# rfonod/geo-trax

Measured on AMD Instinct MI355X. Metric: 4K frames/sec through detect+stabilize+track, higher is better.
Workload: dtype f32 (split-f16x3 MFMA)

## Files before the change

geo-trax_amd/csrc/conv_igemm_split.hip:

```cpp
#include <hip/hip_runtime.h>
#include <hip/hip_fp16.h>

#include <cmath>

#include "conv_split_device.hpp"

namespace gtx {

namespace {

#define GTXS_MFMA(a, b, c) __builtin_amdgcn_mfma_f32_32x32x16_f16(a, b, c, 0, 0, 0)

#ifndef GTXS_DIAG_LOOP_BEGIN
#define GTXS_DIAG_ENTRY()
#define GTXS_DIAG_LOOP_BEGIN()
#define GTXS_DIAG_LOOP_END()
#define GTXS_DIAG_EXIT()
#define GTXS_DIAG_PHASE(K)
#endif

template <int KS, int STRIDE, int WN, int CPR, int WM>
struct SplitTile {
  static constexpr int TH = 8 * WM, TW = 16;
  static constexpr int BN = 32 * WN;
  static constexpr int PAD = KS / 2;
  static constexpr int PH = (TH - 1) * STRIDE + KS;
  static constexpr int PW = (TW - 1) * STRIDE + KS;
  static constexpr int NPIX = PH * PW;
  static constexpr int NCH = 2 * CPR;
  static constexpr int RB = NCH * 16;
  static constexpr int KC = 8 * CPR;
  static constexpr int PATCH_UNITS = NPIX * CPR;
  static constexpr int PATCH_SLOTS = (PATCH_UNITS + 255) / 256;
  static constexpr int W_CHUNKS = KS * KS * BN * NCH;
  static constexpr int W_SLOTS = (W_CHUNKS + 255) / 256;
  static constexpr int PATCH_BYTES = NPIX * RB;
  static constexpr int STAGE_BYTES = PATCH_BYTES + KS * KS * BN * RB;
  static constexpr int EPI_PITCH = epi_pitch(BN), EPI_BYTES = epi_bytes(BN);
  static constexpr int LDS_BYTES = STAGE_BYTES > EPI_BYTES ? STAGE_BYTES : EPI_BYTES;
  static constexpr int ROWS_PER_BANKROW = 256 / RB;
  static __host__ __device__ constexpr int swz(int row) { return (row / ROWS_PER_BANKROW) & (NCH - 1); }
};

__device__ __forceinline__ floatx4 acc_group(const floatx16 a, const int g4) { return floatx4{a[4 * g4], a[4 * g4 + 1], a[4 * g4 + 2], a[4 * g4 + 3]}; }
__device__ __forceinline__ void set_acc_group(floatx16& a, const int g4, const floatx4 v) {
#pragma unroll
  for (int k = 0; k < 4; ++k) a[4 * g4 + k] = v[k];
}

struct FrontTile {
  static constexpr int PH = 17, PW = 33, NPIX = PH * PW;
  static constexpr int IH = 2 * PH + 1, IW = 2 * PW + 1;
  static constexpr int IN_PIX = IH * IW;
  static constexpr int IN_SLOTS = (IN_PIX + 255) / 256;
  static constexpr int IN_BYTES = IN_PIX * 16;
  static constexpr int TILES = (NPIX + 15) / 16;
  static constexpr int LUT_BYTES = 256 * 4;
};

template <int KS, int STRIDE, int WN, int CPR, int WM, int FRONT>
constexpr int split_lds_bytes() {
  using Tile = SplitTile<KS, STRIDE, WN, CPR, WM>;
  if (!FRONT) return Tile::LDS_BYTES;
  const int wreg = Tile::STAGE_BYTES - Tile::PATCH_BYTES > FrontTile::IN_BYTES ? Tile::STAGE_BYTES - Tile::PATCH_BYTES : FrontTile::IN_BYTES;
  const int stage = Tile::PATCH_BYTES + wreg;
  return (stage > Tile::EPI_BYTES ? stage : Tile::EPI_BYTES) + FrontTile::LUT_BYTES;
}

template <int KS, int STRIDE, int WN, int CPR, int WM>
constexpr int split_min_waves() {
  if (WM == 2) return 2;
  if (KS == 3) return STRIDE == 1 ? 3 : 2;
  return WN == 1 ? 5 : 4;
}

template <int KS, int STRIDE, int WN, int CPR, int WM, int FRONT>
__device__ __forceinline__ void conv_split_body(const ConvGroup& g) {
  using Tile = SplitTile<KS, STRIDE, WN, CPR, WM>;
  static_assert(!FRONT || (KS == 3 && STRIDE == 2 && WM == 1 && CPR == 2), "front stage: 3x3 stride 2, 16-channel chunks");
  constexpr int TH = Tile::TH, TW = Tile::TW, BN = Tile::BN, PW = Tile::PW, RB = Tile::RB, KC = Tile::KC;

  extern __shared__ __attribute__((aligned(16))) char smem[];
  char* lds_patch = smem;
  char* lds_w = smem + Tile::PATCH_BYTES;

  GTXS_DIAG_ENTRY()
  const int tid = threadIdx.x;
  const int lane = tid & 63;
  const int wave = __builtin_amdgcn_readfirstlane(tid >> 6);

  ConvProblem P;
  int ct, n, oy0, ox0;
  if (!conv_block_decode<TH, TW>(g, P, ct, n, oy0, ox0)) return;
  const int iy0 = oy0 * STRIDE - Tile::PAD, ix0 = ox0 * STRIDE - Tile::PAD;

  const float* __restrict__ in = static_cast<const float*>(P.in);
  const float* __restrict__ in2 = static_cast<const float*>(P.in2);
  const int nchunks = P.Cin / KC;
  constexpr int c_begin = 0;
  const int c_end = nchunks;

  long goff[Tile::PATCH_SLOTS];
  long goff2[Tile::PATCH_SLOTS];
  int loff[Tile::PATCH_SLOTS];
  int lchk[Tile::PATCH_SLOTS];
  if constexpr (FRONT == 0) {
#pragma unroll
  for (int s = 0; s < Tile::PATCH_SLOTS; ++s) {
    const int qid = tid + 256 * s;
    const int p = qid / CPR, c = qid % CPR;
    const int py = p / PW, px = p - py * PW;
    const int iy = iy0 + py, ix = ix0 + px;
    const bool used = qid < Tile::PATCH_UNITS;
    const bool inb = used && iy >= 0 && iy < P.H && ix >= 0 && ix < P.W;
    goff[s] = inb ? ((long)(n * P.H + iy) * P.W + ix) * P.in_cstride + P.in_coff + c * 8 : -1;
    goff2[s] = (KS == 1 && inb) ? ((long)(n * (P.H >> 1) + (iy >> 1)) * (P.W >> 1) + (ix >> 1)) * P.in2_cstride + P.in2_coff + c * 8 : -1;
    loff[s] = used ? p * RB + ((c ^ Tile::swz(p)) << 4) : -1;
    lchk[s] = used ? p * RB + (((CPR + c) ^ Tile::swz(p)) << 4) : -1;
  }
  }
  const uint4* __restrict__ wsrc =
      reinterpret_cast<const uint4*>(P.wpack) + (size_t)ct * nchunks * Tile::W_CHUNKS + tid;

  const int prow = lane & 31, h = lane >> 5;
  const int tcol = prow & 15;
  const int trow0 = 2 * WM * wave + (prow >> 4);
  const int p0 = trow0 * STRIDE * PW + tcol * STRIDE;
  constexpr int PSUB = 2 * STRIDE * PW;

  uint4 pre_a[Tile::PATCH_SLOTS], pre_b[Tile::PATCH_SLOTS];
  uint4 pre_w[Tile::W_SLOTS];
#define GTXS_PREFETCH(CHUNK)                                                                 \
  {                                                                                          \
    const int c0__ = (CHUNK) * KC;                                                           \
    const bool up__ = KS == 1 && c0__ < P.c_split;    \
    if constexpr (FRONT == 0) {                           \
    _Pragma("unroll") for (int s = 0; s < Tile::PATCH_SLOTS; ++s) {                          \
      uint4 va__ = make_uint4(0, 0, 0, 0), vb__ = make_uint4(0, 0, 0, 0);                    \
      if (goff[s] >= 0) {                                                                    \
        const uint4* src__ = reinterpret_cast<const uint4*>(up__ ? in2 + goff2[s] + c0__ : in + goff[s] + c0__); \
        va__ = src__[0];                                                                     \
        vb__ = src__[1];                                                                     \
      }                                                                                      \
      pre_a[s] = va__;                                                                       \
      pre_b[s] = vb__;                                                                       \
    }                                                                                        \
    }                                                                                        \
    const uint4* w__ = wsrc + (size_t)(CHUNK) * Tile::W_CHUNKS;                              \
    _Pragma("unroll") for (int s = 0; s < Tile::W_SLOTS; ++s) {                              \
      uint4 v__ = make_uint4(0, 0, 0, 0);                                                    \
      if (Tile::W_CHUNKS % 256 == 0 || tid + 256 * s < Tile::W_CHUNKS) v__ = w__[256 * s];  \
      pre_w[s] = v__;                                                                        \
    }                                                                                        \
  }
#define GTXS_COMMIT()                                                                        \
  {                                                                                          \
    if constexpr (FRONT == 0) {                                                                  \
    _Pragma("unroll") for (int s = 0; s < Tile::PATCH_SLOTS; ++s) {                          \
      if (loff[s] >= 0) {                               \
        *reinterpret_cast<uint4*>(lds_patch + loff[s]) = pre_a[s];                           \
        *reinterpret_cast<uint4*>(lds_patch + lchk[s]) = pre_b[s];                           \
      }                                                                                      \
    }                                                                                        \
    }                                                                                        \
    _Pragma("unroll") for (int s = 0; s < Tile::W_SLOTS; ++s) {                              \
      if (Tile::W_CHUNKS % 256 == 0 || tid + 256 * s < Tile::W_CHUNKS)                       \
        *reinterpret_cast<uint4*>(lds_w + (tid + 256 * s) * 16) = pre_w[s];                  \
    }                                                                                        \
  }

  constexpr int FN = FRONT > 0 ? FRONT : 1;
  unsigned f_raw[FrontTile::IN_SLOTS];
  uint2 f_wh[FN][3], f_wl[FN][3];
  float4 f_bias[FN];
  uint2 f_keep[FN > 1 ? FrontTile::TILES / 4 : 1][2];
  char* const f_stage = lds_w;
  unsigned* const f_lut = reinterpret_cast<unsigned*>(smem + split_lds_bytes<KS, STRIDE, WN, CPR, WM, FRONT>() - FrontTile::LUT_BYTES);
  int f_toff[3];
  if constexpr (FRONT > 0) {
    const unsigned* __restrict__ img = static_cast<const unsigned*>(P.front_img) + (size_t)n * P.front_h * P.front_w_px;
    const int gy0 = 2 * iy0 - 1, gx0 = 2 * ix0 - 1;
#pragma unroll
    for (int s = 0; s < FrontTile::IN_SLOTS; ++s) {
      const int i = tid + 256 * s;
      const int r = i / FrontTile::IW, c = i - r * FrontTile::IW;
      const int gy = gy0 + r, gx = gx0 + c;
      f_raw[s] = (i < FrontTile::IN_PIX && gy >= 0 && gy < P.front_h && gx >= 0 && gx < P.front_w_px) ? img[gy * P.front_w_px + gx] : 0u;
    }
#pragma unroll
    for (int c = 0; c < FN; ++c) {
      const uint2* fw = static_cast<const uint2*>(P.front_w) + (size_t)c * (3 * 2 * 64) + lane;
#pragma unroll
      for (int s = 0; s < 3; ++s) {
        f_wh[c][s] = fw[(2 * s + 0) * 64];
        f_wl[c][s] = fw[(2 * s + 1) * 64];
      }
      f_bias[c] = *reinterpret_cast<const float4*>(P.front_bias + c * KC + 4 * (lane >> 4));
    }
#pragma unroll
    for (int s = 0; s < 3; ++s) {
      const int tap = min(4 * s + (lane >> 4), 8);
      f_toff[s] = ((tap / 3) * FrontTile::IW + tap % 3) * 16;
    }
    {
      const float f = (float)tid / 255.f;
      const _Float16 hi = (_Float16)f, lo = (_Float16)(f - (float)hi);
      f_lut[tid] = (unsigned)__builtin_bit_cast(unsigned short, hi) | ((unsigned)__builtin_bit_cast(unsigned short, lo) << 16);
    }
  }
#define GTXS_FRONT_EPI(ACC, BIAS, HV, LV)                                                    \
  {                                                                                          \
     \
    float2v v__[2] = {silu2(__builtin_elementwise_fma(float2v{(ACC)[0], (ACC)[1]}, float2v{P.front_scale, P.front_scale}, float2v{(BIAS).x, (BIAS).y})), \
                      silu2(__builtin_elementwise_fma(float2v{(ACC)[2], (ACC)[3]}, float2v{P.front_scale, P.front_scale}, float2v{(BIAS).z, (BIAS).w}))}; \
    if (!in__) v__[0] = v__[1] = float2v{0.f, 0.f};                                          \
    bool sat__ = false;                                                                      \
    split4(v__, HV, LV, sat__);                                                              \
  }
#define GTXS_FRONT_PUT(T, HV, LV)                                                            \
  {                                                                                          \
    const int qq__ = min((wave + 4 * (T)) * 16 + (lane & 15), FrontTile::NPIX - 1);          \
    const int cg__ = lane >> 4;                               \
    char* row__ = lds_patch + qq__ * RB + (cg__ & 1) * 8;                                    \
    *reinterpret_cast<uint2*>(row__ + (((cg__ >> 1) ^ Tile::swz(qq__)) << 4)) = (HV);        \
    *reinterpret_cast<uint2*>(row__ + (((CPR + (cg__ >> 1)) ^ Tile::swz(qq__)) << 4)) = (LV); \
  }
#define GTXS_FRONT_STAGE()                                                                   \
  {                                                                                          \
    unsigned e__[FrontTile::IN_SLOTS][3];            \
    _Pragma("unroll") for (int s = 0; s < FrontTile::IN_SLOTS; ++s) {                        \
      const unsigned px__ = f_raw[s];                                                        \
      e__[s][0] = f_lut[px__ & 255u]; e__[s][1] = f_lut[(px__ >> 8) & 255u]; e__[s][2] = f_lut[(px__ >> 16) & 255u]; \
    }                                                                                        \
    _Pragma("unroll") for (int s = 0; s < FrontTile::IN_SLOTS; ++s) {                        \
      const int i__ = tid + 256 * s;                                                         \
      if (FrontTile::IN_PIX % 256 == 0 || i__ < FrontTile::IN_PIX)                           \
        *reinterpret_cast<uint4*>(f_stage + i__ * 16) =                                      \
            make_uint4((e__[s][0] & 0xffffu) | (e__[s][1] << 16), e__[s][2] & 0xffffu, (e__[s][0] >> 16) | (e__[s][1] & 0xffff0000u), e__[s][2] >> 16); \
    }                                                                                        \
    __syncthreads();                                                                         \
  }
#define GTXS_FRONT_X(T)                               \
  {                                                                                          \
    const int qc__ = min((wave + 4 * (T)) * 16 + (lane & 15), FrontTile::NPIX - 1);    \
    const int py__ = qc__ / FrontTile::PW, px__ = qc__ - py__ * FrontTile::PW;               \
    const char* src__ = f_stage + (2 * py__ * FrontTile::IW + 2 * px__) * 16;                \
    _Pragma("unroll") for (int s = 0; s < 3; ++s) f_x[(T) % 3][s] = *reinterpret_cast<const uint4*>(src__ + f_toff[s]); \
    const int sy__ = iy0 + py__, sx__ = ix0 + px__;                                          \
    f_in[(T) % 3] = sy__ >= 0 && sy__ < P.H && sx__ >= 0 && sx__ < P.W;    \
  }
#define GTXS_FRONT_M(T)                                        \
  {                                                                                          \
    _Pragma("unroll") for (int c = 0; c < FN; ++c) f_a[(T) % 2][c] = floatx4{0.f, 0.f, 0.f, 0.f}; \
    _Pragma("unroll") for (int s = 0; s < 3; ++s) {                                          \
      const uint4 x__ = f_x[(T) % 3][s];                                                     \
      const uint2 xh2__ = make_uint2(x__.x, x__.y), xl2__ = make_uint2(x__.z, x__.w);        \
      const half4 xh__ = *reinterpret_cast<const half4*>(&xh2__), xl__ = *reinterpret_cast<const half4*>(&xl2__); \
      _Pragma("unroll") for (int c = 0; c < FN; ++c) {                                       \
        const half4 wh__ = *reinterpret_cast<const half4*>(&f_wh[c][s]), wl__ = *reinterpret_cast<const half4*>(&f_wl[c][s]); \
        f_a[(T) % 2][c] = __builtin_amdgcn_mfma_f32_16x16x16f16(wl__, xh__, f_a[(T) % 2][c], 0, 0, 0); \
        f_a[(T) % 2][c] = __builtin_amdgcn_mfma_f32_16x16x16f16(wh__, xl__, f_a[(T) % 2][c], 0, 0, 0); \
        f_a[(T) % 2][c] = __builtin_amdgcn_mfma_f32_16x16x16f16(wh__, xh__, f_a[(T) % 2][c], 0, 0, 0); \
      }                                                                                      \
    }                                                                                        \
  }
#define GTXS_FRONT_TILES()                                                                   \
  {                                                                                          \
    constexpr int NT__ = FrontTile::TILES / 4;                                               \
    uint4 f_x[3][3];                                                                         \
    bool f_in[3];                                                                            \
    floatx4 f_a[2][FN];                                                                      \
    GTXS_FRONT_X(0)                                                                          \
    GTXS_FRONT_X(1)                                                                          \
    GTXS_FRONT_M(0)                                                                          \
    _Pragma("unroll") for (int t__ = 0; t__ < NT__; ++t__) {                                 \
      __builtin_amdgcn_sched_barrier(0);                                                     \
      if (t__ + 2 < NT__) GTXS_FRONT_X(t__ + 2)                                              \
      if (t__ + 1 < NT__) GTXS_FRONT_M(t__ + 1)                                              \
      const bool in__ = f_in[t__ % 3];                                                       \
      uint2 hv0__, lv0__;                                                                    \
      GTXS_FRONT_EPI(f_a[t__ % 2][0], f_bias[0], hv0__, lv0__)                               \
      GTXS_FRONT_PUT(t__, hv0__, lv0__)                                                      \
      if constexpr (FN > 1) GTXS_FRONT_EPI(f_a[t__ % 2][FN - 1], f_bias[FN - 1], f_keep[t__][0], f_keep[t__][1]) \
      if (t__ + 1 < NT__) {                                                                  \
        _Pragma("unroll") for (int i__ = 0; i__ < 9 * FN; ++i__) {                           \
          __builtin_amdgcn_sched_group_barrier(0x008, 1, 0);                                 \
          __builtin_amdgcn_sched_group_barrier(0x002, 4, 0);                                 \
        }                                                                                    \
      }                                                                                      \
      __builtin_amdgcn_sched_barrier(0);                                                     \
    }                                                                                        \
  }

  float4 b4[WN][4];
#define GTXS_LOAD_BIAS()                                                                     \
  {                                                                                          \
    _Pragma("unroll") for (int j = 0; j < WN; ++j)                                           \
      _Pragma("unroll") for (int g4 = 0; g4 < 4; ++g4) b4[j][g4] = make_float4(0.f, 0.f, 0.f, 0.f); \
    if (P.bias) {                              \
      const float* __restrict__ bias_p = P.bias + ct * BN + 4 * (lane >> 5);                 \
      _Pragma("unroll") for (int j = 0; j < WN; ++j)                                         \
        _Pragma("unroll") for (int g4 = 0; g4 < 4; ++g4) b4[j][g4] = *reinterpret_cast<const float4*>(bias_p + 32 * j + 8 * g4);    \
    }                                                                                        \
  }
  if constexpr (FRONT > 0) {
    __syncthreads();
    GTXS_FRONT_STAGE()
    GTXS_PREFETCH(c_begin)
    GTXS_LOAD_BIAS()
    GTXS_FRONT_TILES()
  } else {
    GTXS_PREFETCH(c_begin)
    GTXS_LOAD_BIAS()
  }
#undef GTXS_LOAD_BIAS

  floatx16 acc[WM][WN];
  {
    const float inv_sc = __builtin_amdgcn_rcpf(P.acc_scale);
#pragma unroll
    for (int j = 0; j < WN; ++j)
#pragma unroll
      for (int g4 = 0; g4 < 4; ++g4)
#pragma unroll
        for (int m = 0; m < WM; ++m) set_acc_group(acc[m][j], g4, acc_start(b4[j][g4], inv_sc));
  }

  constexpr int NSTEP = KS * KS * (CPR / 2);
  half8 bh[2][WM], bl[2][WM], ah[2][WN], al[2][WN];
#define GTXS_LOAD_FRAGS(STEP, SLOT)                                                            \
    {                                                                                          \
      const int tap__ = (STEP) / (CPR / 2), ks__ = (STEP) % (CPR / 2);                         \
      const int c__ = 2 * ks__ + h;                                                            \
      _Pragma("unroll") for (int m = 0; m < WM; ++m) {                                         \
        const int p__ = p0 + m * PSUB + (tap__ / KS) * PW + (tap__ % KS);                      \
        const char* pr__ = lds_patch + p__ * RB;                                               \
        bh[SLOT][m] = *reinterpret_cast<const half8*>(pr__ + ((c__ ^ Tile::swz(p__)) << 4));   \
        bl[SLOT][m] = *reinterpret_cast<const half8*>(pr__ + (((CPR + c__) ^ Tile::swz(p__)) << 4)); \
      }                                                                                        \
      _Pragma("unroll") for (int j = 0; j < WN; ++j) {                                         \
        const int nrow__ = 32 * j + prow;                                                      \
        const char* wr__ = lds_w + (tap__ * BN + nrow__) * RB;                                 \
        ah[SLOT][j] = *reinterpret_cast<const half8*>(wr__ + ((c__ ^ Tile::swz(nrow__)) << 4)); \
        al[SLOT][j] = *reinterpret_cast<const half8*>(wr__ + (((CPR + c__) ^ Tile::swz(nrow__)) << 4)); \
      }                                                                                        \
    }
#define GTXS_MATRIX_PHASE()                                                                    \
    GTXS_LOAD_FRAGS(0, 0)                                                                      \
    _Pragma("unroll") for (int st = 0; st < NSTEP; ++st) {                                     \
      __builtin_amdgcn_sched_barrier(0);                                                       \
      if (st + 1 < NSTEP) {                                                                    \
        if (st & 1) GTXS_LOAD_FRAGS(st + 1, 0) else GTXS_LOAD_FRAGS(st + 1, 1)                 \
      }                                                                                        \
      _Pragma("unroll") for (int m = 0; m < WM; ++m)                                           \
        _Pragma("unroll") for (int j = 0; j < WN; ++j) {                                       \
                                                 \
          acc[m][j] = GTXS_MFMA(al[st & 1][j], bh[st & 1][m], acc[m][j]); \
          acc[m][j] = GTXS_MFMA(ah[st & 1][j], bl[st & 1][m], acc[m][j]); \
          acc[m][j] = GTXS_MFMA(ah[st & 1][j], bh[st & 1][m], acc[m][j]); \
        }                                                                                      \
                         \
      _Pragma("unroll") for (int i__ = 0; i__ < 3 * WM * WN; ++i__) {                          \
        __builtin_amdgcn_sched_group_barrier(0x008, 1, 0);                    \
        __builtin_amdgcn_sched_group_barrier(0x100, 1, 0);                                     \
      }                                                                                        \
      __builtin_amdgcn_sched_barrier(0);                                                       \
    }
  constexpr int W2_CHUNKS = BN * BN * 4 / 16, W2_SLOTS = (KS == 3 && STRIDE == 2 && WM == 1) ? (W2_CHUNKS + 255) / 256 : 1;
  uint4 w2r[W2_SLOTS];
  if constexpr (KS == 3 && STRIDE == 2 && WM == 1) {
    if (P.post_w != nullptr) {
#pragma unroll
      for (int i = 0; i < W2_SLOTS; ++i)
        w2r[i] = tid + 256 * i < W2_CHUNKS ? static_cast<const uint4*>(P.post_w)[tid + 256 * i] : make_uint4(0, 0, 0, 0);
    }
  }
  GTXS_DIAG_LOOP_BEGIN()
  for (int chunk = c_begin; chunk < c_end; ++chunk) {
    __syncthreads();
    if constexpr (FRONT > 1) {
      if (chunk != c_begin) {
        _Pragma("unroll") for (int t = 0; t < FrontTile::TILES / 4; ++t) GTXS_FRONT_PUT(t, f_keep[t][0], f_keep[t][1])
      }
    }
    GTXS_COMMIT()
    __syncthreads();
    if (chunk + 1 < c_end) GTXS_PREFETCH(chunk + 1)
    GTXS_MATRIX_PHASE()
    GTXS_DIAG_PHASE(7)
  }
  GTXS_DIAG_LOOP_END()
#undef GTXS_MATRIX_PHASE
#undef GTXS_LOAD_FRAGS
#undef GTXS_FRONT_STAGE
#undef GTXS_FRONT_TILES
#undef GTXS_FRONT_M
#undef GTXS_FRONT_X
#undef GTXS_FRONT_PUT
#undef GTXS_FRONT_EPI

  bool post = false;
  if constexpr (KS == 3 && STRIDE == 2 && WM == 1) {
    if (P.post_w != nullptr) {
      post = true;
      constexpr int PITCH = Tile::EPI_PITCH;
      constexpr int W2_OFF = 4 * 32 * PITCH;
      static_assert(W2_OFF + W2_CHUNKS * 16 <= Tile::LDS_BYTES, "post stage: the 1x1 weights do not fit behind the staging rows");
      float4 b2[WN][4];
#pragma unroll
      for (int j = 0; j < WN; ++j)
#pragma unroll
        for (int g4 = 0; g4 < 4; ++g4)
          b2[j][g4] = P.post_bias ? *reinterpret_cast<const float4*>(P.post_bias + 32 * j + 8 * g4 + 4 * h) : make_float4(0.f, 0.f, 0.f, 0.f);
      __syncthreads();
      char* stg = smem + wave * (32 * PITCH);
      bool sat_y = false;
#pragma unroll
      for (int j = 0; j < WN; ++j)
#pragma unroll
        for (int g4 = 0; g4 < 4; ++g4) {
          const int cl = 32 * j + 8 * g4 + 4 * h;
          epilogue_fragment<32>(acc_group(acc[0][j], g4), P.acc_scale, P.act, false, nullptr, false, stg + prow * PITCH + cl * 4, sat_y);
        }
      flag_saturation(P.sat_flag, sat_y, lane);
#pragma unroll
      for (int i = 0; i < W2_SLOTS; ++i)
        if (tid + 256 * i < W2_CHUNKS) *reinterpret_cast<uint4*>(smem + W2_OFF + (tid + 256 * i) * 16) = w2r[i];
      __syncthreads();
      const float inv2 = __builtin_amdgcn_rcpf(P.post_scale);
#pragma unroll
      for (int j = 0; j < WN; ++j)
#pragma unroll
        for (int g4 = 0; g4 < 4; ++g4) set_acc_group(acc[0][j], g4, acc_start(b2[j][g4], inv2));
      constexpr int K2 = BN / 32;
#pragma unroll
      for (int k2 = 0; k2 < K2; ++k2)
#pragma unroll
        for (int ks = 0; ks < 2; ++ks) {
          const int grp = 2 * (2 * k2 + ks) + h;
          const half8 yh = *reinterpret_cast<const half8*>(stg + prow * PITCH + grp * 32);
          const half8 yl = *reinterpret_cast<const half8*>(stg + prow * PITCH + grp * 32 + 16);
#pragma unroll
          for (int j = 0; j < WN; ++j) {
            const int nrow = 32 * j + prow, sw = swz128(nrow), ci = 2 * ks + h;
            const char* wr = smem + W2_OFF + (k2 * BN + nrow) * 128;
            const half8 wh = *reinterpret_cast<const half8*>(wr + ((ci ^ sw) << 4));
            const half8 wl = *reinterpret_cast<const half8*>(wr + (((4 + ci) ^ sw) << 4));
            acc[0][j] = GTXS_MFMA(wl, yh, acc[0][j]);
            acc[0][j] = GTXS_MFMA(wh, yl, acc[0][j]);
            acc[0][j] = GTXS_MFMA(wh, yh, acc[0][j]);
          }
        }
    }
  }

  const float sc = post ? P.post_scale : P.acc_scale;
  const int cvalid = P.Cout - ct * BN;
  const bool plain = P.out_plain != 0, has_res = P.res != nullptr;
  const int act = post ? P.post_act : P.act;
  bool sat = false;
  __syncthreads();
#pragma unroll
  for (int m = 0; m < WM; ++m) {
    constexpr int PITCH = Tile::EPI_PITCH;
    char* stg = smem + wave * (32 * PITCH);
    const float* __restrict__ res = residual_row(P, n, oy0 + trow0 + 2 * m, ox0 + tcol, ct * BN);
#pragma unroll
    for (int j = 0; j < WN; ++j) {
#pragma unroll
      for (int g4 = 0; g4 < 4; ++g4) {
        const int cl = 32 * j + 8 * g4 + 4 * h;
        epilogue_fragment<32>(acc_group(acc[m][j], g4), sc, act, has_res, (res && cl < cvalid) ? res + cl : nullptr, plain,
                              stg + prow * PITCH + cl * 4, sat);
      }
    }
    store_runs<BN>(stg, P, n, ct, oy0 + 2 * (WM * wave + m), ox0, cvalid, lane);
  }
  flag_saturation(P.sat_flag, sat, lane);
  GTXS_DIAG_EXIT()
}

template <int KS, int STRIDE, int WN, int CPR, int WM>
__global__ __attribute__((amdgpu_flat_work_group_size(1, 256), amdgpu_waves_per_eu((split_min_waves<KS, STRIDE, WN, CPR, WM>()))))
void conv_igemm_split_kernel(const ConvGroup g) {
  conv_split_body<KS, STRIDE, WN, CPR, WM, 0>(g);
}

template <int WN, int NCH>
__global__ __attribute__((amdgpu_flat_work_group_size(1, 256), amdgpu_waves_per_eu(2)))
void conv_front_split_kernel(const ConvGroup g) {
  conv_split_body<3, 2, WN, 2, 1, NCH>(g);
}

template <int KS, int STRIDE, int WN, int CPR, int WM>
void launch_t(const ConvGroup& g, hipStream_t stream) {
  using Tile = SplitTile<KS, STRIDE, WN, CPR, WM>;
  launch_conv_group<conv_igemm_split_kernel<KS, STRIDE, WN, CPR, WM>>(g, 256, Tile::LDS_BYTES, stream);
}

template <int WN, int NCH>
void launch_front_t(const ConvGroup& g, hipStream_t stream) {
  constexpr int lds = split_lds_bytes<3, 2, WN, 2, 1, NCH>();
  static_assert(FrontTile::TILES % 4 == 0 && 2 * lds <= 160 * 1024, "front stage: 9 patch tiles per wave, two workgroups per CU");
  static const int pad = [] { const char* e = getenv("GTX_FRONT_LDS_PAD"); return e ? std::max(0, std::min(atoi(e), 160 * 1024 - lds)) : 0; }();
  launch_conv_group<conv_front_split_kernel<WN, NCH>>(g, 256, lds + pad, stream);
}

}

std::vector<uint8_t> pack_conv_weights_split(const float* w, int cout, int cin, const ConvConfig& cfg, float* acc_scale) {
  const int cpr = cfg.kc / 8, nch = 2 * cpr, rb = nch * 16, rpb = 256 / rb, taps = cfg.ks * cfg.ks;
  const int n_ct = (cout + cfg.bn - 1) / cfg.bn, nchunks = cin / cfg.kc;
  float wmax = 0.f;
  const size_t nw = (size_t)cout * taps * cin;
  for (size_t i = 0; i < nw; ++i) wmax = std::max(wmax, std::fabs(w[i]));
  int shift = 0;
  if (wmax > 0.f && std::isfinite(wmax)) {
    int e;
    std::frexp(wmax, &e);
    shift = 14 - e;
    shift = std::max(-100, std::min(100, shift));
  }
  const float up = std::ldexp(1.f, shift);
  *acc_scale = std::ldexp(1.f, -shift);
  std::vector<uint8_t> out((size_t)n_ct * cfg.bn * taps * cin * 4);
  parallel_for(n_ct * nchunks, [&](int job) {
    const int ct = job / nchunks, ch = job % nchunks;
    for (int tap = 0; tap < taps; ++tap)
      for (int n = 0; n < cfg.bn; ++n) {
        const int sw = (n / rpb) & (nch - 1);
        const size_t row16 = ((((size_t)ct * nchunks + ch) * taps + tap) * cfg.bn + n) * nch;
        for (int c = 0; c < cpr; ++c)
          for (int e = 0; e < 8; ++e) {
            const int ci = ch * cfg.kc + c * 8 + e;
            const float v = ct * cfg.bn + n < cout ? w[((size_t)(ct * cfg.bn + n) * taps + tap) * cin + ci] * up : 0.f;
            const _Float16 hi = (_Float16)v;
            const _Float16 lo = (_Float16)(v - (float)hi);
            memcpy(&out[(row16 + (size_t)(c ^ sw)) * 16 + e * 2], &hi, 2);
            memcpy(&out[(row16 + (size_t)((cpr + c) ^ sw)) * 16 + e * 2], &lo, 2);
          }
      }
  });
  return out;
}

std::vector<uint16_t> pack_front_weights_split(const float* w27 , int c0, float* acc_scale) {
  const int chunks = (c0 + 15) / 16;
  float wmax = 0.f;
  for (int i = 0; i < 27 * c0; ++i) wmax = std::max(wmax, std::fabs(w27[i]));
  int shift = 0;
  if (wmax > 0.f && std::isfinite(wmax)) {
    int e;
    std::frexp(wmax, &e);
    shift = std::max(-100, std::min(100, 14 - e));
  }
  const float up = std::ldexp(1.f, shift);
  *acc_scale = std::ldexp(1.f, -shift);
  std::vector<uint16_t> out((size_t)chunks * 3 * 2 * 64 * 4, 0);
  for (int ch = 0; ch < chunks; ++ch)
    for (int s = 0; s < 3; ++s)
      for (int lane = 0; lane < 64; ++lane) {
        const int co = ch * 16 + (lane & 15), tap = 4 * s + (lane >> 4);
        for (int c = 0; c < 3; ++c) {
          const float v = (tap < 9 && co < c0) ? w27[(size_t)(tap * 3 + c) * c0 + co] * up : 0.f;
          const _Float16 hi = (_Float16)v, lo = (_Float16)(v - (float)hi);
          memcpy(&out[((((size_t)ch * 3 + s) * 2 + 0) * 64 + lane) * 4 + c], &hi, 2);
          memcpy(&out[((((size_t)ch * 3 + s) * 2 + 1) * 64 + lane) * 4 + c], &lo, 2);
        }
      }
  return out;
}

void conv_split_launch(const ConvGroup& g, const ConvConfig& c, hipStream_t s) {
  for (int i = 0; i < g.count; ++i)
    GTX_CHECK(g.p[i].post_w == nullptr || (c.ks == 3 && c.stride == 2 && c.th == 8 && g.p[i].Cout == c.bn && !g.p[i].res),
              "conv: the fused 1x1 post stage needs a 3x3 stride-2 launch whose cout tile holds every channel (Cout %d, tile %d)", g.p[i].Cout, c.bn);
  const int cpr = c.kc / 8, wn = c.bn / 32, wm = c.th / 8;
  if (g.p[0].front_img != nullptr) {
    const ConvProblem& p = g.p[0];
    GTX_CHECK(g.count == 1 && c.ks == 3 && c.stride == 2 && cpr == 2 && wm == 1 && (wn == 1 || wn == 2) && p.Cout <= c.bn &&
                  p.front_w && p.front_bias && p.front_h == 2 * p.H && p.front_w_px == 2 * p.W,
              "conv: the front stage needs a single 3x3 stride-2 launch with one cout tile on a stem output of half the image size");
    if (wn == 1 && p.Cin == 16) return launch_front_t<1, 1>(g, s);
    if (wn == 2 && p.Cin == 32) return launch_front_t<2, 2>(g, s);
    fail(-3, "conv: no front-stage kernel for %d -> %d channels", p.Cin, p.Cout);
  }
#define GTX_CASE(KS, ST, WN, CPR, WM) \
  if (c.ks == KS && c.stride == ST && wn == WN && cpr == CPR && wm == WM) return launch_t<KS, ST, WN, CPR, WM>(g, s);
  GTX_CASE(3, 1, 1, 2, 1) GTX_CASE(3, 1, 2, 2, 1) GTX_CASE(3, 2, 1, 2, 1) GTX_CASE(3, 2, 2, 2, 1)
  GTX_CASE(1, 1, 1, 4, 1) GTX_CASE(1, 1, 2, 4, 1) GTX_CASE(1, 1, 1, 2, 1) GTX_CASE(1, 1, 2, 2, 1)

#undef GTX_CASE
  fail(-3, "conv (split-f16x3): no kernel for ks=%d stride=%d bn=%d kc=%d th=%d", c.ks, c.stride, c.bn, c.kc, c.th);
}

}
```

geo-trax_amd/csrc/conv_k32_split.hip:

```cpp
#include <hip/hip_runtime.h>
#include <hip/hip_fp16.h>

#include "conv_split_device.hpp"

namespace gtx {

namespace {

#define GTXK_MFMA(a, b, c) __builtin_amdgcn_mfma_f32_16x16x32_f16(a, b, c, 0, 0, 0)

struct K32Tile {
  static constexpr int TH = 8, TW = 16, BN = 64, KC = 32, CPR = 4, NCH = 8, RB = 128;
  static constexpr int PH = TH + 2, PW = TW + 2, NPIX = PH * PW;
  static constexpr int PATCH_UNITS = NPIX * CPR;
  static constexpr int PATCH_SLOTS = (PATCH_UNITS + 255) / 256;
  static constexpr int PATCH_BYTES = NPIX * RB;
  static constexpr int WROW_CHUNKS = 3 * BN * NCH;
  static constexpr int W_SLOTS = WROW_CHUNKS / 256;
  static constexpr int WROW_BYTES = WROW_CHUNKS * 16;
  static constexpr int STAGE_BYTES = PATCH_BYTES + WROW_BYTES;
  static constexpr int LDS_BYTES = STAGE_BYTES > epi_bytes(BN) ? STAGE_BYTES : epi_bytes(BN);
};
static_assert(3 * K32Tile::LDS_BYTES <= 160 * 1024, "three workgroups per CU");

__global__ __attribute__((amdgpu_flat_work_group_size(1, 256), amdgpu_waves_per_eu(3)))
void conv_k32_split_kernel(const ConvGroup g) {
  using Tile = K32Tile;
  constexpr int PW = Tile::PW, RB = Tile::RB, BN = Tile::BN, CPR = Tile::CPR;
  extern __shared__ __attribute__((aligned(16))) char smem[];
  char* lds_patch = smem;
  char* lds_w = smem + Tile::PATCH_BYTES;

  const int tid = threadIdx.x;
  const int lane = tid & 63;
  const int wave = __builtin_amdgcn_readfirstlane(tid >> 6);

  ConvProblem P;
  int ct, n, oy0, ox0;
  if (!conv_block_decode<Tile::TH, Tile::TW>(g, P, ct, n, oy0, ox0)) return;
  const int iy0 = oy0 - 1, ix0 = ox0 - 1;

  const float* __restrict__ in = static_cast<const float*>(P.in);
  const int nchunks = P.Cin / Tile::KC;

  int goff[Tile::PATCH_SLOTS];
  int loff[Tile::PATCH_SLOTS];
#pragma unroll
  for (int s = 0; s < Tile::PATCH_SLOTS; ++s) {
    const int qid = tid + 256 * s;
    const int p = qid / CPR, c = qid % CPR;
    const int py = p / PW, px = p - py * PW;
    const int iy = iy0 + py, ix = ix0 + px;
    const bool used = qid < Tile::PATCH_UNITS;
    const bool inb = used && iy >= 0 && iy < P.H && ix >= 0 && ix < P.W;
    goff[s] = inb ? ((n * P.H + iy) * P.W + ix) * P.in_cstride + P.in_coff + c * 8 : -1;
    loff[s] = used ? p * RB + ((c ^ swz128(p)) << 4) : -1;
  }
  const uint4* __restrict__ wsrc = reinterpret_cast<const uint4*>(P.wpack) + (size_t)ct * nchunks * (3 * Tile::WROW_CHUNKS) + tid;

  const int col = lane & 15, kg = lane >> 4;
  const int p0 = (2 * wave) * PW + col;

  uint4 pre_a[Tile::PATCH_SLOTS], pre_b[Tile::PATCH_SLOTS];
  uint4 pw0, pw1, pw2, pw3, pw4, pw5;
  static_assert(Tile::W_SLOTS == 6, "six weight slots");
#define GTXK_PREFETCH_PATCH(CHUNK)                                                           \
  {                                                                                          \
    const int c0__ = (CHUNK) * Tile::KC;                                                     \
    _Pragma("unroll") for (int s = 0; s < Tile::PATCH_SLOTS; ++s) {                          \
      uint4 va__ = make_uint4(0, 0, 0, 0), vb__ = make_uint4(0, 0, 0, 0);                    \
      if (goff[s] >= 0) {                                                                    \
        const uint4* src__ = reinterpret_cast<const uint4*>(in + goff[s] + c0__);            \
        va__ = src__[0];                                                                     \
        vb__ = src__[1];                                                                     \
      }                                                                                      \
      pre_a[s] = va__;                                                                       \
      pre_b[s] = vb__;                                                                       \
    }                                                                                        \
  }
#define GTXK_PREFETCH_W(ROWIDX)                            \
  {                                                                                          \
    const uint4* w__ = wsrc + (size_t)(ROWIDX) * Tile::WROW_CHUNKS;                          \
    pw0 = w__[0]; pw1 = w__[256]; pw2 = w__[512]; pw3 = w__[768]; pw4 = w__[1024]; pw5 = w__[1280]; \
  }
#define GTXK_COMMIT_PATCH()                                                                  \
  {                                                                                          \
    _Pragma("unroll") for (int s = 0; s < Tile::PATCH_SLOTS; ++s) {                          \
      if (loff[s] >= 0) {                                                                    \
        *reinterpret_cast<uint4*>(lds_patch + loff[s]) = pre_a[s];                           \
        *reinterpret_cast<uint4*>(lds_patch + (loff[s] ^ (CPR << 4))) = pre_b[s];                           \
      }                                                                                      \
    }                                                                                        \
  }
#define GTXK_COMMIT_W()                                                                      \
  {                                                                                          \
    uint4* d__ = reinterpret_cast<uint4*>(lds_w) + tid;                                      \
    d__[0] = pw0; d__[256] = pw1; d__[512] = pw2; d__[768] = pw3; d__[1024] = pw4; d__[1280] = pw5; \
  }

  GTXK_PREFETCH_PATCH(0)
  GTXK_PREFETCH_W(0)

  floatx4 acc[4][2];
  {
    const float inv_sc = __builtin_amdgcn_rcpf(P.acc_scale);
#pragma unroll
    for (int a = 0; a < 4; ++a) {
      float4 b = make_float4(0.f, 0.f, 0.f, 0.f);
      if (P.bias) b = *reinterpret_cast<const float4*>(P.bias + ct * BN + 16 * a + 4 * kg);
#pragma unroll
      for (int m = 0; m < 2; ++m) acc[a][m] = acc_start(b, inv_sc);
    }
  }

  half8 bh[2][2], bl[2][2];
  half8 ah[2], al[2];
#define GTXK_LOAD_B(KY, KX, SLOT, Q)                                                           \
    {                                                                                          \
      const int p__ = p0 + (((Q) >> 1) + (KY)) * PW + (KX);                                    \
      const char* pr__ = lds_patch + p__ * RB;                                                 \
      if (((Q) & 1) == 0) bh[SLOT][(Q) >> 1] = *reinterpret_cast<const half8*>(pr__ + ((kg ^ swz128(p__)) << 4)); \
      else bl[SLOT][(Q) >> 1] = *reinterpret_cast<const half8*>(pr__ + (((CPR + kg) ^ swz128(p__)) << 4)); \
    }
#define GTXK_LOAD_A(KX, A, SLOT)                                                               \
    {                                                                                          \
      const int nrow__ = 16 * (A) + col;                                                       \
      const char* wr__ = lds_w + ((KX) * BN + nrow__) * RB;                                    \
      ah[SLOT] = *reinterpret_cast<const half8*>(wr__ + ((kg ^ swz128(nrow__)) << 4));     \
      al[SLOT] = *reinterpret_cast<const half8*>(wr__ + (((CPR + kg) ^ swz128(nrow__)) << 4)); \
    }
#define GTXK_UNIT(KY, U, LAST_ROW)                                                             \
    {                                                                                          \
      constexpr int kx__ = (U) / 4, a__ = (U) % 4;                                             \
      constexpr int bs__ = ((KY) * 3 + kx__) & 1;                                              \
      __builtin_amdgcn_sched_barrier(0);                                                       \
      if ((U) + 1 < 12) GTXK_LOAD_A(((U) + 1) / 4, ((U) + 1) % 4, ((U) + 1) & 1)               \
      if (kx__ < 2) GTXK_LOAD_B(KY, kx__ + 1, bs__ ^ 1, a__)                                   \
      else if (!(LAST_ROW)) GTXK_LOAD_B((KY) + 1, 0, bs__ ^ 1, a__)                            \
      acc[a__][0] = GTXK_MFMA(al[(U) & 1], bh[bs__][0], acc[a__][0]);                          \
      acc[a__][1] = GTXK_MFMA(al[(U) & 1], bh[bs__][1], acc[a__][1]);                          \
      acc[a__][0] = GTXK_MFMA(ah[(U) & 1], bl[bs__][0], acc[a__][0]);                          \
      acc[a__][1] = GTXK_MFMA(ah[(U) & 1], bl[bs__][1], acc[a__][1]);                          \
      acc[a__][0] = GTXK_MFMA(ah[(U) & 1], bh[bs__][0], acc[a__][0]);                          \
      acc[a__][1] = GTXK_MFMA(ah[(U) & 1], bh[bs__][1], acc[a__][1]);                          \
      _Pragma("unroll") for (int i__ = 0; i__ < 3; ++i__) {                                    \
        __builtin_amdgcn_sched_group_barrier(0x008, 1, 0);                                     \
        __builtin_amdgcn_sched_group_barrier(0x100, 1, 0);                                     \
        __builtin_amdgcn_sched_group_barrier(0x008, 1, 0);                                     \
      }                                                                                        \
      __builtin_amdgcn_sched_barrier(0);                                                       \
    }
#define GTXK_ROW(KY, LAST_ROW)                                                                 \
    GTXK_LOAD_A(0, 0, 0)                                                                       \
    GTXK_UNIT(KY, 0, LAST_ROW) GTXK_UNIT(KY, 1, LAST_ROW) GTXK_UNIT(KY, 2, LAST_ROW) GTXK_UNIT(KY, 3, LAST_ROW)   \
    GTXK_UNIT(KY, 4, LAST_ROW) GTXK_UNIT(KY, 5, LAST_ROW) GTXK_UNIT(KY, 6, LAST_ROW) GTXK_UNIT(KY, 7, LAST_ROW)   \
    GTXK_UNIT(KY, 8, LAST_ROW) GTXK_UNIT(KY, 9, LAST_ROW) GTXK_UNIT(KY, 10, LAST_ROW) GTXK_UNIT(KY, 11, LAST_ROW)

  for (int chunk = 0; chunk < nchunks; ++chunk) {
    __syncthreads();
    GTXK_COMMIT_PATCH()
    GTXK_COMMIT_W()
    __syncthreads();
    GTXK_PREFETCH_W(3 * chunk + 1)
    GTXK_LOAD_B(0, 0, 0, 0) GTXK_LOAD_B(0, 0, 0, 1) GTXK_LOAD_B(0, 0, 0, 2) GTXK_LOAD_B(0, 0, 0, 3)
    GTXK_ROW(0, false)
    __syncthreads();
    GTXK_COMMIT_W()
    __syncthreads();
    GTXK_PREFETCH_W(3 * chunk + 2)
    GTXK_ROW(1, false)
    __syncthreads();
    GTXK_COMMIT_W()
    __syncthreads();
    if (chunk + 1 < nchunks) {
      GTXK_PREFETCH_PATCH(chunk + 1)
      GTXK_PREFETCH_W(3 * chunk + 3)
    }
    GTXK_ROW(2, true)
  }
#undef GTXK_ROW
#undef GTXK_UNIT
#undef GTXK_LOAD_A
#undef GTXK_LOAD_B

  epilogue_k32(acc, P, smem, ct, n, oy0, ox0, wave, lane);
}

}

void conv_k32_launch(const ConvGroup& g, const ConvConfig& c, hipStream_t stream) {
  GTX_CHECK(c.ks == 3 && c.stride == 1 && c.bn == K32Tile::BN && c.kc == K32Tile::KC && c.th == 8,
            "conv (K32 form): 3x3 stride 1, 64-cout tiles, 32-channel chunks (ks=%d stride=%d bn=%d kc=%d)", c.ks, c.stride, c.bn, c.kc);
  for (int i = 0; i < g.count; ++i)
    GTX_CHECK(g.p[i].Cin % K32Tile::KC == 0 && g.p[i].post_w == nullptr && g.p[i].front_img == nullptr && g.p[i].c_split == 0,
              "conv (K32 form): Cin %d must be a multiple of 32 and the launch a plain 3x3 layer", g.p[i].Cin);
  launch_conv_group<conv_k32_split_kernel>(g, 256, K32Tile::LDS_BYTES, stream);
}

}
```

geo-trax_amd/csrc/conv_k32s2_split.hip:

```cpp
#include <hip/hip_runtime.h>
#include <hip/hip_fp16.h>

#include "conv_split_device.hpp"

namespace gtx {

namespace {

#define GTXS_MFMA(a, b, c) __builtin_amdgcn_mfma_f32_16x16x32_f16(a, b, c, 0, 0, 0)

struct K32S2Tile {
  static constexpr int TH = 8, TW = 16, BN = 64, KC = 32, CPR = 4, NCH = 8, RB = 128;
  static constexpr int PROWS = TH + 1;
  static constexpr int PW = 2 * TW + 1, NEVEN = TW + 1;
  static constexpr int NPIX = PROWS * PW;
  static constexpr int PATCH_UNITS = NPIX * CPR;
  static constexpr int PATCH_SLOTS = (PATCH_UNITS + 255) / 256;
  static constexpr int PATCH_BYTES = NPIX * RB;
  static constexpr int WROW_CHUNKS = 3 * BN * NCH;
  static constexpr int W_SLOTS = WROW_CHUNKS / 256;
  static constexpr int WROW_BYTES = WROW_CHUNKS * 16;
  static constexpr int STAGE_BYTES = PATCH_BYTES + WROW_BYTES;
  static constexpr int LDS_BYTES = STAGE_BYTES > epi_bytes(BN) ? STAGE_BYTES : epi_bytes(BN);
};
static_assert(2 * K32S2Tile::LDS_BYTES <= 160 * 1024, "two workgroups per CU");

__global__ __attribute__((amdgpu_flat_work_group_size(1, 256), amdgpu_waves_per_eu(2)))
void conv_k32s2_split_kernel(const ConvGroup g) {
  using Tile = K32S2Tile;
  constexpr int PW = Tile::PW, RB = Tile::RB, BN = Tile::BN, CPR = Tile::CPR;
  extern __shared__ __attribute__((aligned(16))) char smem[];
  char* lds_patch = smem;
  char* lds_w = smem + Tile::PATCH_BYTES;

  const int tid = threadIdx.x;
  const int lane = tid & 63;
  const int wave = __builtin_amdgcn_readfirstlane(tid >> 6);

  ConvProblem P;
  int ct, n, oy0, ox0;
  if (!conv_block_decode<Tile::TH, Tile::TW>(g, P, ct, n, oy0, ox0)) return;
  const int iy0 = 2 * oy0 - 1, ix0 = 2 * ox0 - 1;

  const float* __restrict__ in = static_cast<const float*>(P.in);
  const int nchunks = P.Cin / Tile::KC;

  int goff_o[Tile::PATCH_SLOTS], goff_e[Tile::PATCH_SLOTS];
  int loff[Tile::PATCH_SLOTS];
#pragma unroll
  for (int s = 0; s < Tile::PATCH_SLOTS; ++s) {
    const int qid = tid + 256 * s;
    const int p = qid / CPR, c = qid % CPR;
    const int row = p / PW, e = p - row * PW;
    const int px = e < Tile::NEVEN ? 2 * e : 2 * (e - Tile::NEVEN) + 1;
    const int ix = ix0 + px, iyo = iy0 + 2 * row, iye = iyo + 1;
    const bool used = qid < Tile::PATCH_UNITS;
    const bool xin = used && ix >= 0 && ix < P.W;
    goff_o[s] = xin && iyo >= 0 && iyo < P.H ? ((n * P.H + iyo) * P.W + ix) * P.in_cstride + P.in_coff + c * 8 : -1;
    goff_e[s] = xin && row < Tile::TH && iye < P.H ? ((n * P.H + iye) * P.W + ix) * P.in_cstride + P.in_coff + c * 8 : -1;
    loff[s] = used ? p * RB + ((c ^ swz128(p)) << 4) : -1;
  }
  const uint4* __restrict__ wsrc = reinterpret_cast<const uint4*>(P.wpack) + (size_t)ct * nchunks * (3 * Tile::WROW_CHUNKS) + tid;

  const int col = lane & 15, kg = lane >> 4;
  const int p0 = (2 * wave) * PW + col;

  uint4 pre_a[Tile::PATCH_SLOTS], pre_b[Tile::PATCH_SLOTS];
  uint4 pw0, pw1, pw2, pw3, pw4, pw5;
  static_assert(Tile::W_SLOTS == 6, "six weight slots");
#define GTXS_PREFETCH_PATCH(GOFF, CHUNK)                                                     \
  {                                                                                          \
    const int c0__ = (CHUNK) * Tile::KC;                                                     \
    _Pragma("unroll") for (int s = 0; s < Tile::PATCH_SLOTS; ++s) {                          \
      uint4 va__ = make_uint4(0, 0, 0, 0), vb__ = make_uint4(0, 0, 0, 0);                    \
      if (GOFF[s] >= 0) {                                                                    \
        const uint4* src__ = reinterpret_cast<const uint4*>(in + GOFF[s] + c0__);            \
        va__ = src__[0];                                                                     \
        vb__ = src__[1];                                                                     \
      }                                                                                      \
      pre_a[s] = va__;                                                                       \
      pre_b[s] = vb__;                                                                       \
    }                                                                                        \
  }
#define GTXS_PREFETCH_W(ROWIDX)                            \
  {                                                                                          \
    const uint4* w__ = wsrc + (size_t)(ROWIDX) * Tile::WROW_CHUNKS;                          \
    pw0 = w__[0]; pw1 = w__[256]; pw2 = w__[512]; pw3 = w__[768]; pw4 = w__[1024]; pw5 = w__[1280]; \
  }
#define GTXS_COMMIT_PATCH()                                                                  \
  {                                                                                          \
    _Pragma("unroll") for (int s = 0; s < Tile::PATCH_SLOTS; ++s) {                          \
      if (loff[s] >= 0) {                                                                    \
        *reinterpret_cast<uint4*>(lds_patch + loff[s]) = pre_a[s];                           \
        *reinterpret_cast<uint4*>(lds_patch + (loff[s] ^ (CPR << 4))) = pre_b[s];            \
      }                                                                                      \
    }                                                                                        \
  }
#define GTXS_COMMIT_W()                                                                      \
  {                                                                                          \
    uint4* d__ = reinterpret_cast<uint4*>(lds_w) + tid;                                      \
    d__[0] = pw0; d__[256] = pw1; d__[512] = pw2; d__[768] = pw3; d__[1024] = pw4; d__[1280] = pw5; \
  }

  GTXS_PREFETCH_PATCH(goff_o, 0)
  GTXS_PREFETCH_W(0)

  floatx4 acc[4][2];
  {
    const float inv_sc = __builtin_amdgcn_rcpf(P.acc_scale);
#pragma unroll
    for (int a = 0; a < 4; ++a) {
      float4 b = make_float4(0.f, 0.f, 0.f, 0.f);
      if (P.bias) b = *reinterpret_cast<const float4*>(P.bias + ct * BN + 16 * a + 4 * kg);
#pragma unroll
      for (int m = 0; m < 2; ++m) acc[a][m] = acc_start(b, inv_sc);
    }
  }

  half8 bh[2][2], bl[2][2];
  half8 ah[2], al[2];
#define GTXS_LOAD_B(DR, KX, SLOT, Q)                                                           \
    {                                                                                          \
      const int p__ = p0 + (((Q) >> 1) + (DR)) * PW + ((KX) == 1 ? Tile::NEVEN : (KX) >> 1);   \
      const char* pr__ = lds_patch + p__ * RB;                                                 \
      if (((Q) & 1) == 0) bh[SLOT][(Q) >> 1] = *reinterpret_cast<const half8*>(pr__ + ((kg ^ swz128(p__)) << 4)); \
      else bl[SLOT][(Q) >> 1] = *reinterpret_cast<const half8*>(pr__ + (((CPR + kg) ^ swz128(p__)) << 4)); \
    }
#define GTXS_LOAD_A(KX, A, SLOT)                                                               \
    {                                                                                          \
      const int nrow__ = 16 * (A) + col;                                                       \
      const char* wr__ = lds_w + ((KX) * BN + nrow__) * RB;                                    \
      ah[SLOT] = *reinterpret_cast<const half8*>(wr__ + ((kg ^ swz128(nrow__)) << 4));         \
      al[SLOT] = *reinterpret_cast<const half8*>(wr__ + (((CPR + kg) ^ swz128(nrow__)) << 4)); \
    }
#define GTXS_UNIT(ST, DR, U, NEXT_DR)                                                          \
    {                                                                                          \
      constexpr int kx__ = (U) / 4, a__ = (U) % 4;                                             \
      constexpr int bs__ = ((ST) * 3 + kx__) & 1;                                              \
      __builtin_amdgcn_sched_barrier(0);                                                       \
      if ((U) + 1 < 12) GTXS_LOAD_A(((U) + 1) / 4, ((U) + 1) % 4, ((U) + 1) & 1)               \
      if (kx__ < 2) GTXS_LOAD_B(DR, kx__ + 1, bs__ ^ 1, a__)                                   \
      else if ((NEXT_DR) >= 0) GTXS_LOAD_B((NEXT_DR) < 0 ? 0 : (NEXT_DR), 0, bs__ ^ 1, a__)    \
      acc[a__][0] = GTXS_MFMA(al[(U) & 1], bh[bs__][0], acc[a__][0]);                          \
      acc[a__][1] = GTXS_MFMA(al[(U) & 1], bh[bs__][1], acc[a__][1]);                          \
      acc[a__][0] = GTXS_MFMA(ah[(U) & 1], bl[bs__][0], acc[a__][0]);                          \
      acc[a__][1] = GTXS_MFMA(ah[(U) & 1], bl[bs__][1], acc[a__][1]);                          \
      acc[a__][0] = GTXS_MFMA(ah[(U) & 1], bh[bs__][0], acc[a__][0]);                          \
      acc[a__][1] = GTXS_MFMA(ah[(U) & 1], bh[bs__][1], acc[a__][1]);                          \
      _Pragma("unroll") for (int i__ = 0; i__ < 3; ++i__) {                                    \
        __builtin_amdgcn_sched_group_barrier(0x008, 1, 0);                                     \
        __builtin_amdgcn_sched_group_barrier(0x100, 1, 0);                                     \
        __builtin_amdgcn_sched_group_barrier(0x008, 1, 0);                                     \
      }                                                                                        \
      __builtin_amdgcn_sched_barrier(0);                                                       \
    }
#define GTXS_STAGE(ST, DR, NEXT_DR)                                                            \
    GTXS_LOAD_A(0, 0, 0)                                                                       \
    GTXS_UNIT(ST, DR, 0, NEXT_DR) GTXS_UNIT(ST, DR, 1, NEXT_DR) GTXS_UNIT(ST, DR, 2, NEXT_DR) GTXS_UNIT(ST, DR, 3, NEXT_DR)   \
    GTXS_UNIT(ST, DR, 4, NEXT_DR) GTXS_UNIT(ST, DR, 5, NEXT_DR) GTXS_UNIT(ST, DR, 6, NEXT_DR) GTXS_UNIT(ST, DR, 7, NEXT_DR)   \
    GTXS_UNIT(ST, DR, 8, NEXT_DR) GTXS_UNIT(ST, DR, 9, NEXT_DR) GTXS_UNIT(ST, DR, 10, NEXT_DR) GTXS_UNIT(ST, DR, 11, NEXT_DR)

  for (int chunk = 0; chunk < nchunks; ++chunk) {
    __syncthreads();
    GTXS_COMMIT_PATCH()
    GTXS_COMMIT_W()
    __syncthreads();
    GTXS_PREFETCH_W(3 * chunk + 2)
    GTXS_LOAD_B(0, 0, 0, 0) GTXS_LOAD_B(0, 0, 0, 1) GTXS_LOAD_B(0, 0, 0, 2) GTXS_LOAD_B(0, 0, 0, 3)
    GTXS_STAGE(0, 0, 1)
    __syncthreads();
    GTXS_COMMIT_W()
    __syncthreads();
    GTXS_PREFETCH_PATCH(goff_e, chunk)
    GTXS_PREFETCH_W(3 * chunk + 1)
    GTXS_STAGE(1, 1, -1)
    __syncthreads();
    GTXS_COMMIT_PATCH()
    GTXS_COMMIT_W()
    __syncthreads();
    if (chunk + 1 < nchunks) {
      GTXS_PREFETCH_PATCH(goff_o, chunk + 1)
      GTXS_PREFETCH_W(3 * chunk + 3)
    }
    GTXS_LOAD_B(0, 0, 0, 0) GTXS_LOAD_B(0, 0, 0, 1) GTXS_LOAD_B(0, 0, 0, 2) GTXS_LOAD_B(0, 0, 0, 3)
    GTXS_STAGE(2, 0, -1)
  }
#undef GTXS_STAGE
#undef GTXS_UNIT
#undef GTXS_LOAD_A
#undef GTXS_LOAD_B

  epilogue_k32(acc, P, smem, ct, n, oy0, ox0, wave, lane);
}

}

void conv_k32s2_launch(const ConvGroup& g, const ConvConfig& c, hipStream_t stream) {
  GTX_CHECK(c.ks == 3 && c.stride == 2 && c.bn == K32S2Tile::BN && c.kc == K32S2Tile::KC && c.th == 8,
            "conv (K32 stride-2 form): 3x3 stride 2, 64-cout tiles, 32-channel chunks (ks=%d stride=%d bn=%d kc=%d)", c.ks, c.stride, c.bn, c.kc);
  for (int i = 0; i < g.count; ++i)
    GTX_CHECK(g.p[i].Cin % K32S2Tile::KC == 0 && g.p[i].post_w == nullptr && g.p[i].front_img == nullptr && g.p[i].c_split == 0,
              "conv (K32 stride-2 form): Cin %d must be a multiple of 32 and the launch a plain 3x3 layer", g.p[i].Cin);
  launch_conv_group<conv_k32s2_split_kernel>(g, 256, K32S2Tile::LDS_BYTES, stream);
}

}
```

geo-trax_amd/csrc/conv_split_device.hpp:

```cpp
#pragma once
#include <hip/hip_runtime.h>
#include <hip/hip_fp16.h>

#include <mutex>

#include "conv_igemm.hpp"

namespace gtx {

typedef float float2v __attribute__((ext_vector_type(2)));
typedef _Float16 half2v __attribute__((ext_vector_type(2)));
typedef _Float16 half4 __attribute__((ext_vector_type(4)));
typedef _Float16 half8 __attribute__((ext_vector_type(8)));
typedef float floatx4 __attribute__((ext_vector_type(4)));
typedef float floatx16 __attribute__((ext_vector_type(16)));

__device__ __forceinline__ float2v relu2(const float2v v) { return float2v{fmaxf(v.x, 0.f), fmaxf(v.y, 0.f)}; }
__device__ __forceinline__ float2v silu2(const float2v v) {
  const float2v t = v * -1.44269504088896341f;
  const float2v d = float2v{__builtin_amdgcn_exp2f(t.x), __builtin_amdgcn_exp2f(t.y)} + 1.f;
  return v * float2v{__builtin_amdgcn_rcpf(d.x), __builtin_amdgcn_rcpf(d.y)};
}
__device__ __forceinline__ float2v act2(const float2v v, const int act) { return act == 1 ? silu2(v) : act == 2 ? relu2(v) : v; }
__device__ __forceinline__ void split2(const float2v v, unsigned& hi, unsigned& lo, bool& sat) {
  const float2v x = {__builtin_amdgcn_fmed3f(v.x, -65504.f, 65504.f), __builtin_amdgcn_fmed3f(v.y, -65504.f, 65504.f)};
  sat |= x.x != v.x || x.y != v.y;
  const half2v h = __builtin_convertvector(x, half2v);
  const half2v l = __builtin_convertvector(x - __builtin_convertvector(h, float2v), half2v);
  hi = __builtin_bit_cast(unsigned, h);
  lo = __builtin_bit_cast(unsigned, l);
}
__device__ __forceinline__ void split4(const float2v (&v)[2], uint2& hi, uint2& lo, bool& sat) {
  split2(v[0], hi.x, lo.x, sat);
  split2(v[1], hi.y, lo.y, sat);
}
__device__ __forceinline__ floatx4 acc_start(const float4 b, const float inv_sc) {
  return floatx4{b.x * inv_sc, b.y * inv_sc, b.z * inv_sc, b.w * inv_sc};
}

__host__ __device__ constexpr int swz128(int row) { return (row >> 1) & 7; }
__host__ __device__ constexpr int epi_pitch(int bn) { return bn * 4 + 16; }
__host__ __device__ constexpr int epi_bytes(int bn) { return 4 * 32 * epi_pitch(bn); }

template <int TH, int TW>
__device__ __forceinline__ bool conv_block_decode(const ConvGroup& g, ConvProblem& P, int& ct, int& n, int& oy0, int& ox0) {
  const int cnt = g.count;
  int bb[kMaxGroup];
#pragma unroll
  for (int i = 0; i < kMaxGroup; ++i) bb[i] = g.p[i].block_begin;
  const int xcd = blockIdx.x & 7;
  const int L = g.xcd_begin[xcd] + (int)(blockIdx.x >> 3);
  if (L >= g.xcd_begin[xcd + 1]) return false;
  int pi = 0;
#pragma unroll
  for (int i = 1; i < kMaxGroup; ++i)
    if (i < cnt && L >= bb[i]) pi = i;
  P = g.p[pi];
  const int lb = L - P.block_begin;
  ct = lb % P.n_ct;
  const int pt = lb / P.n_ct;
  const int tx = pt % P.tiles_x;
  const int t2 = pt / P.tiles_x;
  const int ty = t2 % P.tiles_y + P.ty_first;
  n = t2 / P.tiles_y;
  oy0 = ty * TH;
  ox0 = tx * TW;
  return true;
}

template <int W>
__device__ __forceinline__ void lane_swap(const unsigned a, const unsigned b, unsigned& lower, unsigned& upper) {
  static_assert(W == 16 || W == 32, "v_permlane16_swap or v_permlane32_swap");
  if constexpr (W == 16) {
    const auto s = __builtin_amdgcn_permlane16_swap(a, b, false, false);
    lower = s[0]; upper = s[1];
  } else {
    const auto s = __builtin_amdgcn_permlane32_swap(a, b, false, false);
    lower = s[0]; upper = s[1];
  }
}
__device__ __forceinline__ const float* residual_row(const ConvProblem& P, const int n, const int oy, const int ox, const int c0) {
  if (!P.res || oy >= P.Ho || ox >= P.Wo) return nullptr;
  return static_cast<const float*>(P.res) + (((size_t)n * P.Ho + oy) * P.Wo + ox) * P.res_cstride + P.res_coff + c0;
}
template <int W>
__device__ __forceinline__ void add_residual(float2v (&v)[2], const float* src) {
  uint4 rc = make_uint4(0, 0, 0, 0);
  if (src) rc = *reinterpret_cast<const uint4*>(src);
  unsigned hw[2], lw[2];
  lane_swap<W>(rc.x, rc.z, hw[0], lw[0]);
  lane_swap<W>(rc.y, rc.w, hw[1], lw[1]);
  const half4 rh = *reinterpret_cast<const half4*>(hw), rl = *reinterpret_cast<const half4*>(lw);
#pragma unroll
  for (int q = 0; q < 2; ++q)
    v[q] += float2v{(float)rh[2 * q], (float)rh[2 * q + 1]} + float2v{(float)rl[2 * q], (float)rl[2 * q + 1]};
}
template <int W>
__device__ __forceinline__ uint4 pair_chunk(const float2v (&v)[2], bool& sat) {
  uint2 hi, lo;
  split4(v, hi, lo, sat);
  uint4 c;
  lane_swap<W>(hi.x, lo.x, c.x, c.z);
  lane_swap<W>(hi.y, lo.y, c.y, c.w);
  return c;
}
template <int W>
__device__ __forceinline__ void epilogue_fragment(const floatx4 a, const float sc, const int act, const bool has_res, const float* res_src,
                                                  const bool plain, char* dst, bool& sat) {
  float2v v[2] = {act2(float2v{a[0], a[1]} * sc, act), act2(float2v{a[2], a[3]} * sc, act)};
  if (has_res) add_residual<W>(v, res_src);
  if (plain) *reinterpret_cast<float4*>(dst) = make_float4(v[0].x, v[0].y, v[1].x, v[1].y);
  else *reinterpret_cast<uint4*>(dst) = pair_chunk<W>(v, sat);
}
template <int BN>
__device__ __forceinline__ void store_runs(const char* stg, const ConvProblem& P, const int n, const int ct, const int py0, const int ox0,
                                           const int cvalid, const int lane) {
  constexpr int LPP = BN / 4;
  constexpr int PPI = 64 / LPP;
#pragma unroll
  for (int it = 0; it < 32 / PPI; ++it) {
    const int p = it * PPI + lane / LPP, q = lane % LPP;
    const int py = py0 + (p >> 4), px = ox0 + (p & 15);
    const uint4 val = *reinterpret_cast<const uint4*>(stg + p * epi_pitch(BN) + q * 16);
    if (py < P.Ho && px < P.Wo && (q >> 1) * 8 < cvalid) {
      float* dst = static_cast<float*>(P.out) + (((size_t)n * P.Ho + py) * P.Wo + px) * P.out_cstride + P.out_coff + ct * BN + q * 4;
      *reinterpret_cast<uint4*>(dst) = val;
    }
  }
}
__device__ __forceinline__ void flag_saturation(int* flag, const bool sat, const int lane) {
  if (flag && __builtin_amdgcn_ballot_w64(sat) != 0 && lane == 0) atomicOr(flag, 1);
}
__device__ __forceinline__ void epilogue_k32(const floatx4 (&acc)[4][2], const ConvProblem& P, char* smem, const int ct, const int n,
                                             const int oy0, const int ox0, const int wave, const int lane) {
  constexpr int BN = 64, PITCH = epi_pitch(BN);
  const int col = lane & 15, kg = lane >> 4;
  const int cvalid = P.Cout - ct * BN;
  const bool plain = P.out_plain != 0, has_res = P.res != nullptr;
  bool sat = false;
  __syncthreads();
  char* stg = smem + wave * (32 * PITCH);
#pragma unroll
  for (int m = 0; m < 2; ++m) {
    const float* __restrict__ res = residual_row(P, n, oy0 + 2 * wave + m, ox0 + col, ct * BN);
#pragma unroll
    for (int a = 0; a < 4; ++a) {
      const int cl = 16 * a + 4 * kg;
      epilogue_fragment<16>(acc[a][m], P.acc_scale, P.act, has_res, (res && cl < cvalid) ? res + cl : nullptr, plain,
                            stg + (16 * m + col) * PITCH + cl * 4, sat);
    }
  }
  store_runs<BN>(stg, P, n, ct, oy0 + 2 * wave, ox0, cvalid, lane);
  flag_saturation(P.sat_flag, sat, lane);
}

template <auto Kernel>
void launch_conv_group(const ConvGroup& g, const int threads, const int lds_bytes, hipStream_t stream) {
  static std::once_flag once;
  std::call_once(once, [&] {
    GTX_HIP(hipFuncSetAttribute(reinterpret_cast<const void*>(Kernel), hipFuncAttributeMaxDynamicSharedMemorySize, lds_bytes));
  });
  hipLaunchKernelGGL(Kernel, dim3(g.grid_blocks), dim3(threads), lds_bytes, stream, g);
  GTX_HIP(hipGetLastError());
}

}
```

geo-trax_amd/csrc/head_sparse.hip:

```cpp
#include <hip/hip_runtime.h>
#include <hip/hip_fp16.h>

#include "conv_split_device.hpp"
#include "det_kernels.hpp"

namespace gtx {

namespace {

#define GTXH_MFMA(a, b, c) __builtin_amdgcn_mfma_f32_16x16x32_f16(a, b, c, 0, 0, 0)

constexpr int kRowBytes = 256;
constexpr int kCandPerWave = 4;
constexpr int kWaveLds = kCandPerWave * 9 * kRowBytes;

__device__ __forceinline__ const char* wrow(const void* w, int step , int row) {
  return static_cast<const char*>(w) + ((size_t)step * 64 + row) * 128;
}

__global__ __launch_bounds__(256) void head_sparse_box_kernel(const SparseBox sb, const NmsBuffers nb, int groups) {
  extern __shared__ __attribute__((aligned(16))) char smem[];
  const int n = blockIdx.y;
  const int l = blockIdx.x / groups, g = blockIdx.x - l * groups;
  const int lane = threadIdx.x & 63;
  const int wave = __builtin_amdgcn_readfirstlane(threadIdx.x >> 6);
  const int cnt = min(nb.lvl_count[n * kMaxLevels + l], nb.lvl_cap);
  const int first = (g * 4 + wave) * kCandPerWave;
  if (first >= cnt) return;
  const SparseBoxLevel& L = sb.lv[l];
  const int col = lane & 15, kg = lane >> 4;
  const int pos = min(col, 8);
  int ci[kCandPerWave], y1[kCandPerWave], x1[kCandPerWave];
  bool valid1[kCandPerWave];
#pragma unroll
  for (int c = 0; c < kCandPerWave; ++c) {
    const int k = min(first + c, cnt - 1);
    ci[c] = __builtin_amdgcn_readfirstlane(nb.lvl_list[((size_t)n * kMaxLevels + l) * nb.lvl_cap + k]);
    const int a = __builtin_amdgcn_readfirstlane(nb.cand_anchor[(size_t)n * nb.cap + ci[c]]);
    const int la = a - L.anchor_begin;
    const int ay = la / L.W, ax = la - ay * L.W;
    y1[c] = ay + pos / 3 - 1;
    x1[c] = ax + pos % 3 - 1;
    valid1[c] = y1[c] >= 0 && y1[c] < L.H && x1[c] >= 0 && x1[c] < L.W;
  }
  const float* __restrict__ in = static_cast<const float*>(L.in) + (size_t)n * L.H * L.W * L.cstride + L.coff + kg * 8;
  char* lds = smem + wave * kWaveLds;

  floatx4 acc[kCandPerWave][4];
  {
    const float inv_sc = __builtin_amdgcn_rcpf(L.sc1);
#pragma unroll
    for (int q = 0; q < 4; ++q) {
      const float4 b = *reinterpret_cast<const float4*>(L.b1 + 16 * q + 4 * kg);
#pragma unroll
      for (int c = 0; c < kCandPerWave; ++c) acc[c][q] = acc_start(b, inv_sc);
    }
  }
  const int nsteps = (L.cin / 32) * 9;
  half8 bh[3][kCandPerWave], bl[3][kCandPerWave], ah[3][4], al[3][4];
#define GTXH_LOAD1(STEP, R)                                                                     \
  {                                                                                             \
    const int ch__ = (STEP) / 9, tap__ = (STEP) - ch__ * 9;                                     \
    _Pragma("unroll") for (int c = 0; c < kCandPerWave; ++c) {                                  \
      const int y__ = y1[c] + tap__ / 3 - 1, x__ = x1[c] + tap__ % 3 - 1;                       \
      uint4 h__ = make_uint4(0, 0, 0, 0), l__ = make_uint4(0, 0, 0, 0);                         \
      if (y__ >= 0 && y__ < L.H && x__ >= 0 && x__ < L.W) {                                     \
        const uint4* s__ = reinterpret_cast<const uint4*>(in + ((size_t)y__ * L.W + x__) * L.cstride + ch__ * 32); \
        h__ = s__[0];                                                                           \
        l__ = s__[1];                                                                           \
      }                                                                                         \
      bh[R][c] = __builtin_bit_cast(half8, h__);                                                \
      bl[R][c] = __builtin_bit_cast(half8, l__);                                                \
    }                                                                                           \
    _Pragma("unroll") for (int q = 0; q < 4; ++q) {                                             \
      const int row__ = 16 * q + col;                                                           \
      const char* w__ = wrow(L.w1, STEP, row__);                                                \
      ah[R][q] = *reinterpret_cast<const half8*>(w__ + ((kg ^ swz128(row__)) << 4));       \
      al[R][q] = *reinterpret_cast<const half8*>(w__ + (((4 + kg) ^ swz128(row__)) << 4)); \
    }                                                                                           \
  }
#define GTXH_STEP1(S, R)                                                                        \
  {                                                                                             \
    if ((S) + 2 < nsteps) GTXH_LOAD1((S) + 2, ((R) + 2) % 3)                                    \
    _Pragma("unroll") for (int c = 0; c < kCandPerWave; ++c)                                    \
      _Pragma("unroll") for (int q = 0; q < 4; ++q) {                                           \
        acc[c][q] = GTXH_MFMA(al[R][q], bh[R][c], acc[c][q]);                                   \
        acc[c][q] = GTXH_MFMA(ah[R][q], bl[R][c], acc[c][q]);                                   \
        acc[c][q] = GTXH_MFMA(ah[R][q], bh[R][c], acc[c][q]);                                   \
      }                                                                                         \
  }
  GTXH_LOAD1(0, 0)
  GTXH_LOAD1(1, 1)
  for (int s = 0; s < nsteps; s += 3) {
    GTXH_STEP1(s, 0)
    GTXH_STEP1(s + 1, 1)
    GTXH_STEP1(s + 2, 2)
  }
#undef GTXH_STEP1
#undef GTXH_LOAD1
  bool sat = false;
#pragma unroll
  for (int c = 0; c < kCandPerWave; ++c)
#pragma unroll
    for (int q = 0; q < 4; ++q) {
      float2v v[2];
#pragma unroll
      for (int e = 0; e < 2; ++e) {
        v[e] = silu2(float2v{acc[c][q][2 * e], acc[c][q][2 * e + 1]} * L.sc1);
        if (!valid1[c]) v[e] = float2v{0.f, 0.f};
      }
      bool s1 = false;
      const uint4 chunk = pair_chunk<16>(v, s1);
      sat |= s1 && col < 9;
      if (col < 9) *reinterpret_cast<uint4*>(lds + (c * 9 + col) * kRowBytes + 64 * q + 16 * kg) = chunk;
    }

  floatx4 acc2[4];
  {
    const float inv_sc = __builtin_amdgcn_rcpf(L.sc2);
#pragma unroll
    for (int q = 0; q < 4; ++q) {
      const float4 b = *reinterpret_cast<const float4*>(L.b2 + 16 * q + 4 * kg);
      acc2[q] = acc_start(b, inv_sc);
    }
  }
  const char* mine = lds + (col & 3) * 9 * kRowBytes;
  half8 wh[3][4], wl[3][4];
#define GTXH_LOAD2(STEP, R)                                                                     \
  _Pragma("unroll") for (int q = 0; q < 4; ++q) {                                               \
    const int row__ = 16 * q + col;                                                             \
    const char* w__ = wrow(L.w2, STEP, row__);                                                  \
    wh[R][q] = *reinterpret_cast<const half8*>(w__ + ((kg ^ swz128(row__)) << 4));         \
    wl[R][q] = *reinterpret_cast<const half8*>(w__ + (((4 + kg) ^ swz128(row__)) << 4));   \
  }
#define GTXH_STEP2(S, R)                                                                        \
  {                                                                                             \
    if ((S) + 2 < 18) GTXH_LOAD2((S) + 2, ((R) + 2) % 3)                                        \
    const int ch__ = (S) / 9, tap__ = (S) - ch__ * 9;                                           \
    const char* r__ = mine + tap__ * kRowBytes + (4 * ch__ + kg) * 32;    \
    const half8 xh__ = *reinterpret_cast<const half8*>(r__), xl__ = *reinterpret_cast<const half8*>(r__ + 16); \
    _Pragma("unroll") for (int q = 0; q < 4; ++q) {                                             \
      acc2[q] = GTXH_MFMA(wl[R][q], xh__, acc2[q]);                                             \
      acc2[q] = GTXH_MFMA(wh[R][q], xl__, acc2[q]);                                             \
      acc2[q] = GTXH_MFMA(wh[R][q], xh__, acc2[q]);                                             \
    }                                                                                           \
  }
  GTXH_LOAD2(0, 0)
  GTXH_LOAD2(1, 1)
#pragma unroll 1
  for (int s = 0; s < 18; s += 3) {
    GTXH_STEP2(s, 0)
    GTXH_STEP2(s + 1, 1)
    GTXH_STEP2(s + 2, 2)
  }
#undef GTXH_STEP2
#undef GTXH_LOAD2
  float* fl = reinterpret_cast<float*>(lds);
  if (col < kCandPerWave) {
#pragma unroll
    for (int q = 0; q < 4; ++q) {
      const float2v v0 = silu2(float2v{acc2[q][0], acc2[q][1]} * L.sc2), v1 = silu2(float2v{acc2[q][2], acc2[q][3]} * L.sc2);
      *reinterpret_cast<float4*>(fl + col * 64 + 16 * q + 4 * kg) = make_float4(v0.x, v0.y, v1.x, v1.y);
    }
  }
#pragma unroll 1
  for (int c = 0; c < kCandPerWave; ++c) {
    if (first + c >= cnt) break;
    float a = L.bb[lane];
    const float* wr = L.wb + lane;
#pragma unroll 8
    for (int k = 0; k < 64; ++k) a = fmaf(fl[c * 64 + k], wr[(size_t)k * 64], a);
    const int anchor = __builtin_amdgcn_readfirstlane(nb.cand_anchor[(size_t)n * nb.cap + ci[c]]);
    const int la = anchor - L.anchor_begin;
    float m = a;
#pragma unroll
    for (int o = 8; o >= 1; o >>= 1) m = fmaxf(m, __shfl_xor(m, o, 64));
    const float e = expf(a - m);
    float se = e, sw = e * (float)(lane & 15);
#pragma unroll
    for (int o = 8; o >= 1; o >>= 1) {
      se += __shfl_xor(se, o, 64);
      sw += __shfl_xor(sw, o, 64);
    }
    const float d = sw / se;
    const float d0 = __shfl(d, 0, 64), d1 = __shfl(d, 16, 64), d2 = __shfl(d, 32, 64), d3 = __shfl(d, 48, 64);
    const float ax = (float)(la % L.W) + 0.5f, ay = (float)(la / L.W) + 0.5f;
    const float bx1 = ax - d0, by1 = ay - d1, bx2 = ax + d2, by2 = ay + d3;
    const float4 b = make_float4((bx1 + bx2) * 0.5f * L.stride, (by1 + by2) * 0.5f * L.stride, (bx2 - bx1) * L.stride, (by2 - by1) * L.stride);
    if (lane == 0) {
      const float hw = b.z / 2.f, hh = b.w / 2.f;
      reinterpret_cast<float4*>(nb.cand_box)[(size_t)n * nb.cap + ci[c]] = make_float4(b.x - hw, b.y - hh, b.x + hw, b.y + hh);
    }
  }
  flag_saturation(sb.sat_flag, sat, lane);
}

}

void launch_head_sparse_box(const SparseBox& sb, int n, const NmsBuffers& nb, hipStream_t s) {
  GTX_CHECK(sb.cap > 0 && nb.lvl_count != nullptr && nb.lvl_list != nullptr && nb.lvl_cap == sb.cap, "sparse box branch: no buffers");
  const int groups = (nb.lvl_cap + 4 * kCandPerWave - 1) / (4 * kCandPerWave);
  hipLaunchKernelGGL(head_sparse_box_kernel, dim3(sb.n_levels * groups, n), dim3(256), 4 * kWaveLds, s, sb, nb, groups);
  GTX_HIP(hipGetLastError());
}

}
```

Baseline: 1176.

## Restructure LDS layouts to cut bank conflicts in k32 and sparse-head kernels

Moves LDS addressing into a shared layout header. By default it switches the k32 convolution patch to a two-plane layout with 64-byte pixel rows and a new XOR swizzle, and pads the sparse-head candidate rows from 256 to 272 bytes. The igemm and epilogue addressing keep their old formulas behind helper functions. The goal is fewer LDS bank-conflict passes on the MFMA operand reads and the staging writes. It also adds a host-side bank-conflict model and a diagnostic tool; the new layouts change LDS footprint slightly and could move conflicts elsewhere.

```diff
diff --git a/geo-trax_amd/csrc/conv_igemm_split.hip b/geo-trax_amd/csrc/conv_igemm_split.hip
--- a/geo-trax_amd/csrc/conv_igemm_split.hip
+++ b/geo-trax_amd/csrc/conv_igemm_split.hip
@@ -38,8 +38,6 @@
   static constexpr int STAGE_BYTES = PATCH_BYTES + KS * KS * BN * RB;
   static constexpr int EPI_PITCH = epi_pitch(BN), EPI_BYTES = epi_bytes(BN);
   static constexpr int LDS_BYTES = STAGE_BYTES > EPI_BYTES ? STAGE_BYTES : EPI_BYTES;
-  static constexpr int ROWS_PER_BANKROW = 256 / RB;
-  static __host__ __device__ constexpr int swz(int row) { return (row / ROWS_PER_BANKROW) & (NCH - 1); }
 };
 
 __device__ __forceinline__ floatx4 acc_group(const floatx16 a, const int g4) { return floatx4{a[4 * g4], a[4 * g4 + 1], a[4 * g4 + 2], a[4 * g4 + 3]}; }
@@ -115,8 +113,8 @@
     const bool inb = used && iy >= 0 && iy < P.H && ix >= 0 && ix < P.W;
     goff[s] = inb ? ((long)(n * P.H + iy) * P.W + ix) * P.in_cstride + P.in_coff + c * 8 : -1;
     goff2[s] = (KS == 1 && inb) ? ((long)(n * (P.H >> 1) + (iy >> 1)) * (P.W >> 1) + (ix >> 1)) * P.in2_cstride + P.in2_coff + c * 8 : -1;
-    loff[s] = used ? p * RB + ((c ^ Tile::swz(p)) << 4) : -1;
-    lchk[s] = used ? p * RB + (((CPR + c) ^ Tile::swz(p)) << 4) : -1;
+    loff[s] = used ? row_off<RB>(p, c) : -1;
+    lchk[s] = used ? row_off<RB>(p, CPR + c) : -1;
   }
   }
   const uint4* __restrict__ wsrc =
@@ -221,9 +219,9 @@
   {                                                                                          \
     const int qq__ = min((wave + 4 * (T)) * 16 + (lane & 15), FrontTile::NPIX - 1);          \
     const int cg__ = lane >> 4;                               \
-    char* row__ = lds_patch + qq__ * RB + (cg__ & 1) * 8;                                    \
-    *reinterpret_cast<uint2*>(row__ + (((cg__ >> 1) ^ Tile::swz(qq__)) << 4)) = (HV);        \
-    *reinterpret_cast<uint2*>(row__ + (((CPR + (cg__ >> 1)) ^ Tile::swz(qq__)) << 4)) = (LV); \
+    char* row__ = lds_patch + (cg__ & 1) * 8;                                                \
+    *reinterpret_cast<uint2*>(row__ + row_off<RB>(qq__, cg__ >> 1)) = (HV);                  \
+    *reinterpret_cast<uint2*>(row__ + row_off<RB>(qq__, CPR + (cg__ >> 1))) = (LV);          \
   }
 #define GTXS_FRONT_STAGE()                                                                   \
   {                                                                                          \
@@ -334,15 +332,14 @@
       const int c__ = 2 * ks__ + h;                                                            \
       _Pragma("unroll") for (int m = 0; m < WM; ++m) {                                         \
         const int p__ = p0 + m * PSUB + (tap__ / KS) * PW + (tap__ % KS);                      \
-        const char* pr__ = lds_patch + p__ * RB;                                               \
-        bh[SLOT][m] = *reinterpret_cast<const half8*>(pr__ + ((c__ ^ Tile::swz(p__)) << 4));   \
-        bl[SLOT][m] = *reinterpret_cast<const half8*>(pr__ + (((CPR + c__) ^ Tile::swz(p__)) << 4)); \
+        bh[SLOT][m] = *reinterpret_cast<const half8*>(lds_patch + row_off<RB>(p__, c__));      \
+        bl[SLOT][m] = *reinterpret_cast<const half8*>(lds_patch + row_off<RB>(p__, CPR + c__)); \
       }                                                                                        \
       _Pragma("unroll") for (int j = 0; j < WN; ++j) {                                         \
         const int nrow__ = 32 * j + prow;                                                      \
-        const char* wr__ = lds_w + (tap__ * BN + nrow__) * RB;                                 \
-        ah[SLOT][j] = *reinterpret_cast<const half8*>(wr__ + ((c__ ^ Tile::swz(nrow__)) << 4)); \
-        al[SLOT][j] = *reinterpret_cast<const half8*>(wr__ + (((CPR + c__) ^ Tile::swz(nrow__)) << 4)); \
+        const char* wr__ = lds_w + tap__ * BN * RB;                                            \
+        ah[SLOT][j] = *reinterpret_cast<const half8*>(wr__ + row_off<RB>(nrow__, c__));        \
+        al[SLOT][j] = *reinterpret_cast<const half8*>(wr__ + row_off<RB>(nrow__, CPR + c__));  \
       }                                                                                        \
     }
 #define GTXS_MATRIX_PHASE()                                                                    \
@@ -420,7 +417,7 @@
 #pragma unroll
         for (int g4 = 0; g4 < 4; ++g4) {
           const int cl = 32 * j + 8 * g4 + 4 * h;
-          epilogue_fragment<32>(acc_group(acc[0][j], g4), P.acc_scale, P.act, false, nullptr, false, stg + prow * PITCH + cl * 4, sat_y);
+          epilogue_fragment<32>(acc_group(acc[0][j], g4), P.acc_scale, P.act, false, nullptr, false, stg + epi_off(BN, prow, cl * 4), sat_y);
         }
       flag_saturation(P.sat_flag, sat_y, lane);
 #pragma unroll
@@ -438,14 +435,14 @@
 #pragma unroll
         for (int ks = 0; ks < 2; ++ks) {
           const int grp = 2 * (2 * k2 + ks) + h;
-          const half8 yh = *reinterpret_cast<const half8*>(stg + prow * PITCH + grp * 32);
-          const half8 yl = *reinterpret_cast<const half8*>(stg + prow * PITCH + grp * 32 + 16);
+          const half8 yh = *reinterpret_cast<const half8*>(stg + epi_off(BN, prow, grp * 32));
+          const half8 yl = *reinterpret_cast<const half8*>(stg + epi_off(BN, prow, grp * 32 + 16));
 #pragma unroll
           for (int j = 0; j < WN; ++j) {
-            const int nrow = 32 * j + prow, sw = swz128(nrow), ci = 2 * ks + h;
-            const char* wr = smem + W2_OFF + (k2 * BN + nrow) * 128;
-            const half8 wh = *reinterpret_cast<const half8*>(wr + ((ci ^ sw) << 4));
-            const half8 wl = *reinterpret_cast<const half8*>(wr + (((4 + ci) ^ sw) << 4));
+            const int nrow = 32 * j + prow, ci = 2 * ks + h;
+            const char* wr = smem + W2_OFF + k2 * BN * 128;
+            const half8 wh = *reinterpret_cast<const half8*>(wr + row128_off(nrow, ci));
+            const half8 wl = *reinterpret_cast<const half8*>(wr + row128_off(nrow, 4 + ci));
             acc[0][j] = GTXS_MFMA(wl, yh, acc[0][j]);
             acc[0][j] = GTXS_MFMA(wh, yl, acc[0][j]);
             acc[0][j] = GTXS_MFMA(wh, yh, acc[0][j]);
@@ -471,7 +468,7 @@
       for (int g4 = 0; g4 < 4; ++g4) {
         const int cl = 32 * j + 8 * g4 + 4 * h;
         epilogue_fragment<32>(acc_group(acc[m][j], g4), sc, act, has_res, (res && cl < cvalid) ? res + cl : nullptr, plain,
-                              stg + prow * PITCH + cl * 4, sat);
+                              stg + epi_off(BN, prow, cl * 4), sat);
       }
     }
     store_runs<BN>(stg, P, n, ct, oy0 + 2 * (WM * wave + m), ox0, cvalid, lane);
diff --git a/geo-trax_amd/csrc/conv_k32_split.hip b/geo-trax_amd/csrc/conv_k32_split.hip
--- a/geo-trax_amd/csrc/conv_k32_split.hip
+++ b/geo-trax_amd/csrc/conv_k32_split.hip
@@ -14,7 +14,7 @@
   static constexpr int PH = TH + 2, PW = TW + 2, NPIX = PH * PW;
   static constexpr int PATCH_UNITS = NPIX * CPR;
   static constexpr int PATCH_SLOTS = (PATCH_UNITS + 255) / 256;
-  static constexpr int PATCH_BYTES = NPIX * RB;
+  static constexpr int PATCH_BYTES = k32_patch_bytes(NPIX);
   static constexpr int WROW_CHUNKS = 3 * BN * NCH;
   static constexpr int W_SLOTS = WROW_CHUNKS / 256;
   static constexpr int WROW_BYTES = WROW_CHUNKS * 16;
@@ -54,7 +54,7 @@
     const bool used = qid < Tile::PATCH_UNITS;
     const bool inb = used && iy >= 0 && iy < P.H && ix >= 0 && ix < P.W;
     goff[s] = inb ? ((n * P.H + iy) * P.W + ix) * P.in_cstride + P.in_coff + c * 8 : -1;
-    loff[s] = used ? p * RB + ((c ^ swz128(p)) << 4) : -1;
+    loff[s] = used ? k32_patch_off(Tile::NPIX, p, c, 0) : -1;
   }
   const uint4* __restrict__ wsrc = reinterpret_cast<const uint4*>(P.wpack) + (size_t)ct * nchunks * (3 * Tile::WROW_CHUNKS) + tid;
 
@@ -88,7 +88,7 @@
     _Pragma("unroll") for (int s = 0; s < Tile::PATCH_SLOTS; ++s) {                          \
       if (loff[s] >= 0) {                                                                    \
         *reinterpret_cast<uint4*>(lds_patch + loff[s]) = pre_a[s];                           \
-        *reinterpret_cast<uint4*>(lds_patch + (loff[s] ^ (CPR << 4))) = pre_b[s];                           \
+        *reinterpret_cast<uint4*>(lds_patch + k32_patch_lo(loff[s])) = pre_b[s];                           \
       }                                                                                      \
     }                                                                                        \
   }
@@ -118,16 +118,15 @@
 #define GTXK_LOAD_B(KY, KX, SLOT, Q)                                                           \
     {                                                                                          \
       const int p__ = p0 + (((Q) >> 1) + (KY)) * PW + (KX);                                    \
-      const char* pr__ = lds_patch + p__ * RB;                                                 \
-      if (((Q) & 1) == 0) bh[SLOT][(Q) >> 1] = *reinterpret_cast<const half8*>(pr__ + ((kg ^ swz128(p__)) << 4)); \
-      else bl[SLOT][(Q) >> 1] = *reinterpret_cast<const half8*>(pr__ + (((CPR + kg) ^ swz128(p__)) << 4)); \
+      if (((Q) & 1) == 0) bh[SLOT][(Q) >> 1] = *reinterpret_cast<const half8*>(lds_patch + k32_patch_off(Tile::NPIX, p__, kg, 0)); \
+      else bl[SLOT][(Q) >> 1] = *reinterpret_cast<const half8*>(lds_patch + k32_patch_off(Tile::NPIX, p__, kg, 1)); \
     }
 #define GTXK_LOAD_A(KX, A, SLOT)                                                               \
     {                                                                                          \
       const int nrow__ = 16 * (A) + col;                                                       \
-      const char* wr__ = lds_w + ((KX) * BN + nrow__) * RB;                                    \
-      ah[SLOT] = *reinterpret_cast<const half8*>(wr__ + ((kg ^ swz128(nrow__)) << 4));     \
-      al[SLOT] = *reinterpret_cast<const half8*>(wr__ + (((CPR + kg) ^ swz128(nrow__)) << 4)); \
+      const char* wr__ = lds_w + (KX) * BN * RB;                                               \
+      ah[SLOT] = *reinterpret_cast<const half8*>(wr__ + row128_off(nrow__, kg));               \
+      al[SLOT] = *reinterpret_cast<const half8*>(wr__ + row128_off(nrow__, CPR + kg));         \
     }
 #define GTXK_UNIT(KY, U, LAST_ROW)                                                             \
     {                                                                                          \
diff --git a/geo-trax_amd/csrc/conv_k32s2_split.hip b/geo-trax_amd/csrc/conv_k32s2_split.hip
--- a/geo-trax_amd/csrc/conv_k32s2_split.hip
+++ b/geo-trax_amd/csrc/conv_k32s2_split.hip
@@ -16,7 +16,7 @@
   static constexpr int NPIX = PROWS * PW;
   static constexpr int PATCH_UNITS = NPIX * CPR;
   static constexpr int PATCH_SLOTS = (PATCH_UNITS + 255) / 256;
-  static constexpr int PATCH_BYTES = NPIX * RB;
+  static constexpr int PATCH_BYTES = k32_patch_bytes(NPIX);
   static constexpr int WROW_CHUNKS = 3 * BN * NCH;
   static constexpr int W_SLOTS = WROW_CHUNKS / 256;
   static constexpr int WROW_BYTES = WROW_CHUNKS * 16;
@@ -58,7 +58,7 @@
     const bool xin = used && ix >= 0 && ix < P.W;
     goff_o[s] = xin && iyo >= 0 && iyo < P.H ? ((n * P.H + iyo) * P.W + ix) * P.in_cstride + P.in_coff + c * 8 : -1;
     goff_e[s] = xin && row < Tile::TH && iye < P.H ? ((n * P.H + iye) * P.W + ix) * P.in_cstride + P.in_coff + c * 8 : -1;
-    loff[s] = used ? p * RB + ((c ^ swz128(p)) << 4) : -1;
+    loff[s] = used ? k32_patch_off(Tile::NPIX, p, c, 0) : -1;
   }
   const uint4* __restrict__ wsrc = reinterpret_cast<const uint4*>(P.wpack) + (size_t)ct * nchunks * (3 * Tile::WROW_CHUNKS) + tid;
 
@@ -92,7 +92,7 @@
     _Pragma("unroll") for (int s = 0; s < Tile::PATCH_SLOTS; ++s) {                          \
       if (loff[s] >= 0) {                                                                    \
         *reinterpret_cast<uint4*>(lds_patch + loff[s]) = pre_a[s];                           \
-        *reinterpret_cast<uint4*>(lds_patch + (loff[s] ^ (CPR << 4))) = pre_b[s];            \
+        *reinterpret_cast<uint4*>(lds_patch + k32_patch_lo(loff[s])) = pre_b[s];            \
       }                                                                                      \
     }                                                                                        \
   }
@@ -122,16 +122,15 @@
 #define GTXS_LOAD_B(DR, KX, SLOT, Q)                                                           \
     {                                                                                          \
       const int p__ = p0 + (((Q) >> 1) + (DR)) * PW + ((KX) == 1 ? Tile::NEVEN : (KX) >> 1);   \
-      const char* pr__ = lds_patch + p__ * RB;                                                 \
-      if (((Q) & 1) == 0) bh[SLOT][(Q) >> 1] = *reinterpret_cast<const half8*>(pr__ + ((kg ^ swz128(p__)) << 4)); \
-      else bl[SLOT][(Q) >> 1] = *reinterpret_cast<const half8*>(pr__ + (((CPR + kg) ^ swz128(p__)) << 4)); \
+      if (((Q) & 1) == 0) bh[SLOT][(Q) >> 1] = *reinterpret_cast<const half8*>(lds_patch + k32_patch_off(Tile::NPIX, p__, kg, 0)); \
+      else bl[SLOT][(Q) >> 1] = *reinterpret_cast<const half8*>(lds_patch + k32_patch_off(Tile::NPIX, p__, kg, 1)); \
     }
 #define GTXS_LOAD_A(KX, A, SLOT)                                                               \
     {                                                                                          \
       const int nrow__ = 16 * (A) + col;                                                       \
-      const char* wr__ = lds_w + ((KX) * BN + nrow__) * RB;                                    \
-      ah[SLOT] = *reinterpret_cast<const half8*>(wr__ + ((kg ^ swz128(nrow__)) << 4));         \
-      al[SLOT] = *reinterpret_cast<const half8*>(wr__ + (((CPR + kg) ^ swz128(nrow__)) << 4)); \
+      const char* wr__ = lds_w + (KX) * BN * RB;                                               \
+      ah[SLOT] = *reinterpret_cast<const half8*>(wr__ + row128_off(nrow__, kg));               \
+      al[SLOT] = *reinterpret_cast<const half8*>(wr__ + row128_off(nrow__, CPR + kg));         \
     }
 #define GTXS_UNIT(ST, DR, U, NEXT_DR)                                                          \
     {                                                                                          \
diff --git a/geo-trax_amd/csrc/conv_split_device.hpp b/geo-trax_amd/csrc/conv_split_device.hpp
--- a/geo-trax_amd/csrc/conv_split_device.hpp
+++ b/geo-trax_amd/csrc/conv_split_device.hpp
@@ -5,6 +5,7 @@
 #include <mutex>
 
 #include "conv_igemm.hpp"
+#include "lds_layout.hpp"
 
 namespace gtx {
 
@@ -38,9 +39,6 @@
   return floatx4{b.x * inv_sc, b.y * inv_sc, b.z * inv_sc, b.w * inv_sc};
 }
 
-__host__ __device__ constexpr int swz128(int row) { return (row >> 1) & 7; }
-__host__ __device__ constexpr int epi_pitch(int bn) { return bn * 4 + 16; }
-__host__ __device__ constexpr int epi_bytes(int bn) { return 4 * 32 * epi_pitch(bn); }
 
 template <int TH, int TW>
 __device__ __forceinline__ bool conv_block_decode(const ConvGroup& g, ConvProblem& P, int& ct, int& n, int& oy0, int& ox0) {
@@ -121,7 +119,7 @@
   for (int it = 0; it < 32 / PPI; ++it) {
     const int p = it * PPI + lane / LPP, q = lane % LPP;
     const int py = py0 + (p >> 4), px = ox0 + (p & 15);
-    const uint4 val = *reinterpret_cast<const uint4*>(stg + p * epi_pitch(BN) + q * 16);
+    const uint4 val = *reinterpret_cast<const uint4*>(stg + epi_off(BN, p, q * 16));
     if (py < P.Ho && px < P.Wo && (q >> 1) * 8 < cvalid) {
       float* dst = static_cast<float*>(P.out) + (((size_t)n * P.Ho + py) * P.Wo + px) * P.out_cstride + P.out_coff + ct * BN + q * 4;
       *reinterpret_cast<uint4*>(dst) = val;
@@ -133,13 +131,13 @@
 }
 __device__ __forceinline__ void epilogue_k32(const floatx4 (&acc)[4][2], const ConvProblem& P, char* smem, const int ct, const int n,
                                              const int oy0, const int ox0, const int wave, const int lane) {
-  constexpr int BN = 64, PITCH = epi_pitch(BN);
+  constexpr int BN = 64;
   const int col = lane & 15, kg = lane >> 4;
   const int cvalid = P.Cout - ct * BN;
   const bool plain = P.out_plain != 0, has_res = P.res != nullptr;
   bool sat = false;
   __syncthreads();
-  char* stg = smem + wave * (32 * PITCH);
+  char* stg = smem + wave * (32 * epi_pitch(BN));
 #pragma unroll
   for (int m = 0; m < 2; ++m) {
     const float* __restrict__ res = residual_row(P, n, oy0 + 2 * wave + m, ox0 + col, ct * BN);
@@ -147,7 +145,7 @@
     for (int a = 0; a < 4; ++a) {
       const int cl = 16 * a + 4 * kg;
       epilogue_fragment<16>(acc[a][m], P.acc_scale, P.act, has_res, (res && cl < cvalid) ? res + cl : nullptr, plain,
-                            stg + (16 * m + col) * PITCH + cl * 4, sat);
+                            stg + epi_off(BN, 16 * m + col, cl * 4), sat);
     }
   }
   store_runs<BN>(stg, P, n, ct, oy0 + 2 * wave, ox0, cvalid, lane);
diff --git a/geo-trax_amd/csrc/diag/lds_conflict_check.cpp b/geo-trax_amd/csrc/diag/lds_conflict_check.cpp
--- /dev/null
+++ b/geo-trax_amd/csrc/diag/lds_conflict_check.cpp
@@ -0,0 +1,294 @@
+#include <cstdio>
+#include <cstdlib>
+#include <cstring>
+#include <string>
+#include <vector>
+
+#include "../lds_bank_model.hpp"
+#include "../lds_layout.hpp"
+
+using namespace gtx;
+using gtx::ldsmodel::Kind;
+using gtx::ldsmodel::Passes;
+
+namespace {
+
+struct Site {
+  std::string kernel, site, kind;
+  bool hot;
+  int instr = 0, passes = 0, minimum = 0, worst = 0;
+};
+std::vector<Site> g_sites;
+
+const char* kind_name(Kind k) {
+  switch (k) {
+    case Kind::ReadB32: return "ds_read_b32";
+    case Kind::ReadB64: return "ds_read_b64";
+    case Kind::ReadB128: return "ds_read_b128";
+    case Kind::WriteB64: return "ds_write_b64";
+    default: return "ds_write_b128";
+  }
+}
+
+struct Acc {
+  Site s;
+  Kind kind;
+  Acc(const char* kernel, const char* site, Kind k, bool hot) : kind(k) {
+    s.kernel = kernel; s.site = site; s.kind = kind_name(k); s.hot = hot;
+  }
+  void add(const int (&addr)[64], uint64_t active = ~0ull) {
+    if (active == 0) return;
+    const Passes p = ldsmodel::lds_passes(kind, addr, active);
+    s.instr += 1; s.passes += p.passes; s.minimum += p.minimum;
+    s.worst = p.worst > s.worst ? p.worst : s.worst;
+  }
+  ~Acc() { g_sites.push_back(s); }
+};
+
+void k32_family(const char* name, bool s2) {
+  const int PW = s2 ? 33 : 18, NPIX = s2 ? 9 * 33 : 10 * 18, BN = 64;
+  const int slots = (NPIX * 4 + 255) / 256;
+  {
+    Acc hi(name, "patch fragment read, hi", Kind::ReadB128, true), lo(name, "patch fragment read, lo", Kind::ReadB128, true);
+    for (int wave = 0; wave < 4; ++wave)
+      for (int ky = 0; ky < 3; ++ky)
+        for (int kx = 0; kx < 3; ++kx)
+          for (int m = 0; m < 2; ++m) {
+            int ah[64], al[64];
+            for (int lane = 0; lane < 64; ++lane) {
+              const int col = lane & 15, kg = lane >> 4;
+              const int p0 = 2 * wave * PW + col;
+              const int p = s2 ? p0 + (m + (ky == 1 ? 1 : 0)) * PW + (kx == 1 ? 17 : kx >> 1) : p0 + (m + ky) * PW + kx;
+              ah[lane] = k32_patch_off(NPIX, p, kg, 0);
+              al[lane] = k32_patch_off(NPIX, p, kg, 1);
+            }
+            hi.add(ah);
+            lo.add(al);
+          }
+  }
+  {
+    Acc a(name, "weight fragment read, hi + lo", Kind::ReadB128, true);
+    for (int rep = 0; rep < 4 * 3; ++rep)
+    for (int kx = 0; kx < 3; ++kx)
+      for (int blk = 0; blk < 4; ++blk)
+        for (int lo = 0; lo < 2; ++lo) {
+          int ad[64];
+          for (int lane = 0; lane < 64; ++lane) ad[lane] = kx * BN * 128 + row128_off(16 * blk + (lane & 15), 4 * lo + (lane >> 4));
+          a.add(ad);
+        }
+  }
+  {
+    Acc a(name, "patch commit, hi + lo", Kind::WriteB128, false);
+    for (int s = 0; s < slots; ++s)
+      for (int wave = 0; wave < 4; ++wave) {
+        int ah[64], al[64];
+        uint64_t act = 0;
+        for (int lane = 0; lane < 64; ++lane) {
+          const int qid = wave * 64 + lane + 256 * s;
+          const int p = qid / 4, c = qid % 4;
+          ah[lane] = al[lane] = 0;
+          if (qid < NPIX * 4) {
+            act |= 1ull << lane;
+            ah[lane] = k32_patch_off(NPIX, p, c, 0);
+            al[lane] = k32_patch_lo(ah[lane]);
+          }
+        }
+        a.add(ah, act);
+        a.add(al, act);
+      }
+  }
+  {
+    Acc a(name, "weight row commit", Kind::WriteB128, false);
+    for (int k = 0; k < 3 * 6; ++k)
+      for (int wave = 0; wave < 4; ++wave) {
+        int ad[64];
+        for (int lane = 0; lane < 64; ++lane) ad[lane] = (wave * 64 + lane + 256 * k) * 16;
+        a.add(ad);
+      }
+  }
+  {
+    Acc w(name, "epilogue staging store", Kind::WriteB128, false), r(name, "epilogue run read", Kind::ReadB128, false);
+    for (int wave = 0; wave < 4; ++wave)
+    for (int m = 0; m < 2; ++m)
+      for (int blk = 0; blk < 4; ++blk) {
+        int ad[64];
+        for (int lane = 0; lane < 64; ++lane) ad[lane] = epi_off(BN, 16 * m + (lane & 15), (16 * blk + 4 * (lane >> 4)) * 4);
+        w.add(ad);
+      }
+    for (int it = 0; it < 4 * 8; ++it) {
+      int ad[64];
+      for (int lane = 0; lane < 64; ++lane) ad[lane] = epi_off(BN, (it % 8) * 4 + lane / 16, (lane % 16) * 16);
+      r.add(ad);
+    }
+  }
+}
+
+template <int KS, int STRIDE, int WN, int CPR, int WM>
+void igemm_family(const char* name) {
+  constexpr int TH = 8 * WM, TW = 16, BN = 32 * WN, PH = (TH - 1) * STRIDE + KS, PW = (TW - 1) * STRIDE + KS, NPIX = PH * PW;
+  constexpr int NCH = 2 * CPR, RB = NCH * 16, UNITS = NPIX * CPR, SLOTS = (UNITS + 255) / 256;
+  constexpr int W_CHUNKS = KS * KS * BN * NCH, W_SLOTS = (W_CHUNKS + 255) / 256, PSUB = 2 * STRIDE * PW;
+  {
+    Acc b(name, "patch fragment read, hi + lo", Kind::ReadB128, true), a(name, "weight fragment read, hi + lo", Kind::ReadB128, true);
+    for (int wave = 0; wave < 4; ++wave)
+      for (int step = 0; step < KS * KS * (CPR / 2); ++step) {
+        const int tap = step / (CPR / 2), ks = step % (CPR / 2);
+        for (int lo = 0; lo < 2; ++lo) {
+          for (int m = 0; m < WM; ++m) {
+            int ad[64];
+            for (int lane = 0; lane < 64; ++lane) {
+              const int prow = lane & 31, h = lane >> 5, c = 2 * ks + h;
+              const int trow0 = 2 * WM * wave + (prow >> 4);
+              const int p = trow0 * STRIDE * PW + (prow & 15) * STRIDE + m * PSUB + (tap / KS) * PW + tap % KS;
+              ad[lane] = row_off<RB>(p, lo * CPR + c);
+            }
+            b.add(ad);
+          }
+          for (int j = 0; j < WN; ++j) {
+              int ad[64];
+              for (int lane = 0; lane < 64; ++lane) ad[lane] = tap * BN * RB + row_off<RB>(32 * j + (lane & 31), lo * CPR + 2 * ks + (lane >> 5));
+              a.add(ad);
+            }
+        }
+      }
+  }
+  {
+    Acc a(name, "patch commit, hi + lo", Kind::WriteB128, false);
+    for (int s = 0; s < SLOTS; ++s)
+      for (int wave = 0; wave < 4; ++wave) {
+        int ah[64], al[64];
+        uint64_t act = 0;
+        for (int lane = 0; lane < 64; ++lane) {
+          const int qid = wave * 64 + lane + 256 * s;
+          ah[lane] = al[lane] = 0;
+          if (qid < UNITS) {
+            act |= 1ull << lane;
+            ah[lane] = row_off<RB>(qid / CPR, qid % CPR);
+            al[lane] = row_off<RB>(qid / CPR, CPR + qid % CPR);
+          }
+        }
+        a.add(ah, act);
+        a.add(al, act);
+      }
+  }
+  {
+    Acc a(name, "weight commit", Kind::WriteB128, false);
+    for (int s = 0; s < W_SLOTS; ++s)
+      for (int wave = 0; wave < 4; ++wave) {
+        int ad[64];
+        uint64_t act = 0;
+        for (int lane = 0; lane < 64; ++lane) {
+          const int i = wave * 64 + lane + 256 * s;
+          ad[lane] = i < W_CHUNKS ? i * 16 : 0;
+          if (i < W_CHUNKS) act |= 1ull << lane;
+        }
+        a.add(ad, act);
+      }
+  }
+  {
+    Acc w(name, "epilogue staging store", Kind::WriteB128, false), r(name, "epilogue run read", Kind::ReadB128, false);
+    for (int rep = 0; rep < 4 * WM; ++rep)
+    for (int j = 0; j < WN; ++j)
+      for (int g4 = 0; g4 < 4; ++g4) {
+        int ad[64];
+        for (int lane = 0; lane < 64; ++lane) ad[lane] = epi_off(BN, lane & 31, (32 * j + 8 * g4 + 4 * (lane >> 5)) * 4);
+        w.add(ad);
+      }
+    constexpr int LPP = BN / 4, PPI = 64 / LPP;
+    for (int it = 0; it < 4 * WM * (32 / PPI); ++it) {
+      int ad[64];
+      for (int lane = 0; lane < 64; ++lane) ad[lane] = epi_off(BN, (it % (32 / PPI)) * PPI + lane / LPP, (lane % LPP) * 16);
+      r.add(ad);
+    }
+  }
+}
+
+void sparse_family() {
+  const char* name = "head_sparse_box_kernel";
+  {
+    Acc w(name, "first-layer pixel store", Kind::WriteB128, false);
+    for (int c = 0; c < 4; ++c)
+      for (int q = 0; q < 4; ++q) {
+        int ad[64];
+        uint64_t act = 0;
+        for (int lane = 0; lane < 64; ++lane) {
+          const int col = lane & 15, kg = lane >> 4;
+          ad[lane] = col < 9 ? sparse_px_off(c, col, 64 * q + 16 * kg) : 0;
+          if (col < 9) act |= 1ull << lane;
+        }
+        w.add(ad, act);
+      }
+  }
+  {
+    Acc r(name, "second-layer pixel read, hi + lo", Kind::ReadB128, true);
+    for (int s = 0; s < 18; ++s)
+      for (int lo = 0; lo < 2; ++lo) {
+        int ad[64];
+        for (int lane = 0; lane < 64; ++lane) ad[lane] = sparse_px_off(lane & 3, s % 9, (4 * (s / 9) + (lane >> 4)) * 32 + 16 * lo);
+        r.add(ad);
+      }
+  }
+  {
+    Acc w(name, "box feature store", Kind::WriteB128, false), r(name, "box feature read (decode, broadcast)", Kind::ReadB32, false);
+    for (int q = 0; q < 4; ++q) {
+      int ad[64];
+      uint64_t act = 0;
+      for (int lane = 0; lane < 64; ++lane) {
+        const int col = lane & 15, kg = lane >> 4;
+        ad[lane] = col < 4 ? (col * 64 + 16 * q + 4 * kg) * 4 : 0;
+        if (col < 4) act |= 1ull << lane;
+      }
+      w.add(ad, act);
+    }
+    for (int c = 0; c < 4; ++c)
+      for (int k = 0; k < 64; ++k) {
+        int ad[64];
+        for (int lane = 0; lane < 64; ++lane) ad[lane] = (c * 64 + k) * 4;
+        r.add(ad);
+      }
+  }
+}
+
+int pattern(int argc, char** argv) {
+  if (argc != 3 + 64) { fprintf(stderr, "usage: --pattern read_b32|read_b64|read_b128|write_b64|write_b128 a0 .. a63\n"); return 2; }
+  const std::string k = argv[2];
+  const Kind kind = k == "read_b32" ? Kind::ReadB32 : k == "read_b64" ? Kind::ReadB64 : k == "read_b128" ? Kind::ReadB128
+                    : k == "write_b64" ? Kind::WriteB64 : Kind::WriteB128;
+  int ad[64];
+  for (int i = 0; i < 64; ++i) ad[i] = atoi(argv[3 + i]);
+  const Passes p = ldsmodel::lds_passes(kind, ad);
+  printf("passes %d minimum %d worst %d\n", p.passes, p.minimum, p.worst);
+  return 0;
+}
+
+}
+
+int main(int argc, char** argv) {
+  if (argc > 1 && !strcmp(argv[1], "--pattern")) return pattern(argc, argv);
+  k32_family("conv_k32_split_kernel", false);
+  k32_family("conv_k32s2_split_kernel", true);
+  igemm_family<1, 1, 2, 4, 1>("conv_igemm_split_kernel<1,1,2,4,1>");
+  igemm_family<3, 2, 2, 2, 1>("conv_igemm_split_kernel<3,2,2,2,1>");
+  igemm_family<3, 1, 1, 2, 1>("conv_igemm_split_kernel<3,1,1,2,1>");
+  sparse_family();
+#ifdef GTX_LDS_PARENT_LAYOUT
+  printf("# layout: parent (128-byte patch rows in the 16x16x32 kernels, 256-byte sparse rows)\n");
+#else
+  printf("# layout: two-plane patch in the 16x16x32 kernels, 272-byte sparse rows\n");
+#endif
+  printf("# one workgroup (the sparse kernel: one wave), one K chunk; passes = LDS-array cycles, min = conflict-free; share = (passes - min) / passes\n");
+  printf("%-36s | %-38s | %-13s | %3s | %5s | %6s | %4s | %5s | %s\n", "kernel", "site", "instruction", "hot", "instr", "passes", "min", "worst", "share");
+  std::string cur;
+  int kp = 0, km = 0;
+  auto flush = [&] {
+    if (!cur.empty()) printf("%-36s | %-38s | %-13s | %3s | %5s | %6d | %4d | %5s | %.3f\n", cur.c_str(), "TOTAL", "", "", "", kp, km, "", kp ? (double)(kp - km) / kp : 0.0);
+  };
+  for (const Site& s : g_sites) {
+    if (s.kernel != cur) { flush(); cur = s.kernel; kp = km = 0; }
+    printf("%-36s | %-38s | %-13s | %3s | %5d | %6d | %4d | %5d | %.3f\n", s.kernel.c_str(), s.site.c_str(), s.kind.c_str(), s.hot ? "yes" : "no", s.instr,
+           s.passes, s.minimum, s.worst, s.passes ? (double)(s.passes - s.minimum) / s.passes : 0.0);
+    kp += s.passes; km += s.minimum;
+  }
+  flush();
+  return 0;
+}
diff --git a/geo-trax_amd/csrc/head_sparse.hip b/geo-trax_amd/csrc/head_sparse.hip
--- a/geo-trax_amd/csrc/head_sparse.hip
+++ b/geo-trax_amd/csrc/head_sparse.hip
@@ -10,9 +10,8 @@
 
 #define GTXH_MFMA(a, b, c) __builtin_amdgcn_mfma_f32_16x16x32_f16(a, b, c, 0, 0, 0)
 
-constexpr int kRowBytes = 256;
 constexpr int kCandPerWave = 4;
-constexpr int kWaveLds = kCandPerWave * 9 * kRowBytes;
+constexpr int kWaveLds = kCandPerWave * kSparseCandPitch;
 
 __device__ __forceinline__ const char* wrow(const void* w, int step , int row) {
   return static_cast<const char*>(w) + ((size_t)step * 64 + row) * 128;
@@ -112,7 +111,7 @@
       bool s1 = false;
       const uint4 chunk = pair_chunk<16>(v, s1);
       sat |= s1 && col < 9;
-      if (col < 9) *reinterpret_cast<uint4*>(lds + (c * 9 + col) * kRowBytes + 64 * q + 16 * kg) = chunk;
+      if (col < 9) *reinterpret_cast<uint4*>(lds + sparse_px_off(c, col, 64 * q + 16 * kg)) = chunk;
     }
 
   floatx4 acc2[4];
@@ -124,7 +123,7 @@
       acc2[q] = acc_start(b, inv_sc);
     }
   }
-  const char* mine = lds + (col & 3) * 9 * kRowBytes;
+  const int mine = col & 3;
   half8 wh[3][4], wl[3][4];
 #define GTXH_LOAD2(STEP, R)                                                                     \
   _Pragma("unroll") for (int q = 0; q < 4; ++q) {                                               \
@@ -137,7 +136,7 @@
   {                                                                                             \
     if ((S) + 2 < 18) GTXH_LOAD2((S) + 2, ((R) + 2) % 3)                                        \
     const int ch__ = (S) / 9, tap__ = (S) - ch__ * 9;                                           \
-    const char* r__ = mine + tap__ * kRowBytes + (4 * ch__ + kg) * 32;    \
+    const char* r__ = lds + sparse_px_off(mine, tap__, (4 * ch__ + kg) * 32);    \
     const half8 xh__ = *reinterpret_cast<const half8*>(r__), xl__ = *reinterpret_cast<const half8*>(r__ + 16); \
     _Pragma("unroll") for (int q = 0; q < 4; ++q) {                                             \
       acc2[q] = GTXH_MFMA(wl[R][q], xh__, acc2[q]);                                             \
diff --git a/geo-trax_amd/csrc/lds_bank_model.hpp b/geo-trax_amd/csrc/lds_bank_model.hpp
--- /dev/null
+++ b/geo-trax_amd/csrc/lds_bank_model.hpp
@@ -0,0 +1,65 @@
+#pragma once
+#include <cstdint>
+
+namespace gtx {
+namespace ldsmodel {
+
+enum class Kind { ReadB32, ReadB64, ReadB128, WriteB64, WriteB128 };
+
+struct KindInfo {
+  int groups, lanes_per_group, dwords, banks;
+};
+constexpr KindInfo kind_info(Kind k) {
+  return k == Kind::ReadB32     ? KindInfo{2, 32, 1, 32}
+         : k == Kind::ReadB64   ? KindInfo{2, 32, 2, 64}
+         : k == Kind::ReadB128  ? KindInfo{4, 16, 4, 64}
+         : k == Kind::WriteB64  ? KindInfo{4, 16, 2, 32}
+                                : KindInfo{8, 8, 4, 32};
+}
+constexpr int group_lane(Kind k, int g, int i) {
+  if (k == Kind::ReadB128) {
+    constexpr int g0[16] = {0, 1, 2, 3, 12, 13, 14, 15, 20, 21, 22, 23, 24, 25, 26, 27};
+    constexpr int g1[16] = {4, 5, 6, 7, 8, 9, 10, 11, 16, 17, 18, 19, 28, 29, 30, 31};
+    return ((g & 1) ? g1[i] : g0[i]) + 32 * (g >> 1);
+  }
+  return g * kind_info(k).lanes_per_group + i;
+}
+
+struct Passes {
+  int passes;
+  int minimum;
+  int worst;
+};
+
+constexpr Passes lds_passes(Kind kind, const int (&addr)[64], uint64_t active = ~0ull) {
+  const KindInfo ki = kind_info(kind);
+  Passes r{0, 0, 0};
+  for (int g = 0; g < ki.groups; ++g) {
+    int dw[16 * 4 * 2] = {};
+    int ndw = 0;
+    for (int i = 0; i < ki.lanes_per_group; ++i) {
+      const int lane = group_lane(kind, g, i);
+      if (!((active >> lane) & 1)) continue;
+      for (int d = 0; d < ki.dwords; ++d) {
+        const int w = addr[lane] / 4 + d;
+        bool seen = false;
+        for (int k = 0; k < ndw; ++k) seen = seen || dw[k] == w;
+        if (!seen) dw[ndw++] = w;
+      }
+    }
+    if (ndw == 0) continue;
+    int worst = 0;
+    for (int b = 0; b < ki.banks; ++b) {
+      int n = 0;
+      for (int k = 0; k < ndw; ++k) n += (dw[k] % ki.banks) == b;
+      worst = n > worst ? n : worst;
+    }
+    r.passes += worst;
+    r.minimum += 1;
+    r.worst = worst > r.worst ? worst : r.worst;
+  }
+  return r;
+}
+
+}
+}
diff --git a/geo-trax_amd/csrc/lds_layout.hpp b/geo-trax_amd/csrc/lds_layout.hpp
--- /dev/null
+++ b/geo-trax_amd/csrc/lds_layout.hpp
@@ -0,0 +1,50 @@
+#pragma once
+
+#if defined(__HIPCC__)
+#define GTX_HD __host__ __device__
+#else
+#define GTX_HD
+#endif
+
+namespace gtx {
+
+GTX_HD constexpr int swz128(int row) { return (row >> 1) & 7; }
+GTX_HD constexpr int row128_off(int row, int chunk) { return row * 128 + ((chunk ^ swz128(row)) << 4); }
+template <int RB>
+GTX_HD constexpr int row_off(int row, int chunk) { return row * RB + ((chunk ^ ((row / (256 / RB)) & (RB / 16 - 1))) << 4); }
+GTX_HD constexpr int k32_plane_bytes(int npix) { return (npix * 64 + 255) / 256 * 256; }
+GTX_HD constexpr int k32_patch_bytes(int npix) {
+#ifdef GTX_LDS_PARENT_LAYOUT
+  return npix * 128;
+#else
+  return 2 * k32_plane_bytes(npix);
+#endif
+}
+GTX_HD constexpr int k32_patch_off(int npix, int p, int c, int lo) {
+#ifdef GTX_LDS_PARENT_LAYOUT
+  return row128_off(p, 4 * lo + c);
+#else
+  return (c & 1) * k32_plane_bytes(npix) + p * 64 + ((((c >> 1) + 2 * lo) ^ ((p >> 2) & 3)) << 4);
+#endif
+}
+GTX_HD constexpr int k32_patch_lo(int hi_off) {
+#ifdef GTX_LDS_PARENT_LAYOUT
+  return hi_off ^ 64;
+#else
+  return hi_off ^ 32;
+#endif
+}
+GTX_HD constexpr int epi_pitch(int bn) { return bn * 4 + 16; }
+GTX_HD constexpr int epi_bytes(int bn) { return 4 * 32 * epi_pitch(bn); }
+GTX_HD constexpr int epi_off(int bn, int pixel, int byte) { return pixel * epi_pitch(bn) + byte; }
+
+
+#ifdef GTX_LDS_PARENT_LAYOUT
+constexpr int kSparseRowPitch = 256, kSparseCandPitch = 9 * 256;
+#else
+constexpr int kSparseRowPitch = 272, kSparseCandPitch = 164 * 16;
+#endif
+static_assert(kSparseCandPitch >= 9 * kSparseRowPitch, "a candidate's nine pixel rows");
+GTX_HD constexpr int sparse_px_off(int cand, int pos, int byte) { return cand * kSparseCandPitch + pos * kSparseRowPitch + byte; }
+
+}
```

New measurement: 1174, median of 2. Within noise of the previous version (-0.2%).
